# excamera/alfalfa

Hardware: AMD Instinct MI355X
Metric: 1080p macroblocks/s decode (bit-exact vs reference) (higher is better)
Workload: dtype u8

## Files before the change

### alfalfa_amd/__init__.py

```python
import os as _os

_os.environ.setdefault("GPU_MAX_HW_QUEUES", "16")

from .decoder import AlfalfaError, Context, Decoder, FilePlayer, Parser, Quality, psnr, read_ivf
```

### alfalfa_amd/capi.py

```python
import ctypes as C
import os

import numpy as np

from . import build as _build

AA_OK = 0
ERR_NAMES = {-1: "Invalid", -2: "Unsupported", -3: "LogicError", -4: "OutOfRange", -5: "HipError",
             -6: "NoDevice", -7: "BadArgument", -8: "NoMemory"}

AA_MB_HAS_NONZERO, AA_MB_HAS_Y2, AA_MB_INTER, AA_MB_SKIP, AA_MB_LF_SKIP_INNER = 1, 2, 4, 8, 16

MB_INFO_DTYPE = np.dtype([("y_mode", "u1"), ("uv_mode", "u1"), ("ref_frame", "u1"), ("segment_id", "u1"),
                          ("flags", "u1"), ("lf_level", "u1"), ("split_partition", "u1"), ("reserved", "u1"),
                          ("nz_mask", "<u4"), ("coeff_index", "<u4"), ("u", "u1", (64,))])
assert MB_INFO_DTYPE.itemsize == 80


class FrameHeader(C.Structure):
    _fields_ = [(n, C.c_uint8) for n in (
        "key_frame", "show_frame", "loop_filter_level", "sharpness_level", "num_dct_partitions",
        "segmentation_enabled", "filter_adjustments_enabled", "refresh_last", "refresh_golden",
        "refresh_alternate", "copy_buffer_to_golden", "copy_buffer_to_alternate", "sign_bias_golden",
        "sign_bias_alternate", "q_index", "has_intra_mb")] + [
        ("mb_width", C.c_uint16), ("mb_height", C.c_uint16), ("width", C.c_uint16), ("height", C.c_uint16),
        ("quant", (C.c_uint16 * 6) * 4), ("num_macroblocks", C.c_uint32), ("num_coeff_blocks", C.c_uint32),
        ("num_intra_mbs", C.c_uint32), ("compressed_size", C.c_uint32)]

    def as_dict(self):
        d = {n: getattr(self, n) for n, _ in self._fields_ if n != "quant"}
        d["quant"] = [[self.quant[s][k] for k in range(6)] for s in range(4)]
        return d


class FrameIn(C.Structure):
    _fields_ = [("stream", C.c_void_p), ("data", C.c_char_p), ("size", C.c_size_t)]


class KernelStats(C.Structure):
    _fields_ = [("recon_inter_ms", C.c_double), ("recon_intra_ms", C.c_double), ("loopfilter_ms", C.c_double),
                ("recon_inter_launches", C.c_uint64), ("recon_intra_launches", C.c_uint64),
                ("loopfilter_launches", C.c_uint64), ("macroblocks", C.c_uint64),
                ("parse_headers_ms", C.c_double), ("parse_tokens_ms", C.c_double), ("parse_launches", C.c_uint64),
                ("parsed_macroblocks", C.c_uint64), ("recon_split_ms", C.c_double), ("recon_split_launches", C.c_uint64),
                ("pool_waits", C.c_uint64), ("pool_wait_ms", C.c_double), ("parse_wait_ms", C.c_double),
                ("bind_wait_ms", C.c_double), ("alloc_ms", C.c_double), ("slab_mallocs", C.c_uint64),
                ("token_steps", C.c_uint64), ("token_frames", C.c_uint64), ("worker_launches", C.c_uint64), ("worker_wgs", C.c_uint64),
                ("worker_retires", C.c_uint64), ("heap_grows", C.c_uint64), ("heap_mapped_bytes", C.c_uint64), ("nomem_retries", C.c_uint64), ("frames_evicted", C.c_uint64), ("host_routed_frames", C.c_uint64),
                ("row_handoff_stale_polls", C.c_uint64), ("row_handoff_rereads", C.c_uint64), ("packed_frames", C.c_uint64), ("packed_words", C.c_uint64), ("packed_blocks", C.c_uint64),
                ("host_batch_ms", C.c_double), ("host_batch_parse_wall_ms", C.c_double), ("host_batch_parse_cpu_ms", C.c_double), ("host_batch_arena_ms", C.c_double),
                ("pinned_allocs", C.c_uint64)]


class CtxInfo(C.Structure):
    _fields_ = [(n, C.c_uint64) for n in ("memory_limit_bytes", "pool_bytes", "pool_free_bytes", "pool_pending_bytes", "heap_mapped_bytes", "heap_limit_bytes", "heap_used_bytes",
                                          "pinned_host_bytes")] + [
        (n, C.c_uint32) for n in ("heap_is_virtual", "token_lanes_per_workgroup", "token_workgroups_capacity", "token_workgroups_alive",
                                  "token_lane_lds_bytes", "token_workgroup_lds_bytes", "jobs_waiting", "compute_units")] + [
        ("heap_free_chunks", C.c_int32), ("lanes_starved", C.c_uint32), ("token_profile", C.c_uint64 * 8),
        ("packed_coefficients", C.c_uint32), ("lane_per_partition", C.c_uint32), ("clock_mhz", C.c_uint32), ("host_share_ms", C.c_uint32), ("host_rate_kb_per_ms", C.c_uint32), ("reserved1", C.c_uint32), ("stream_concurrency", C.c_uint32), ("streams_needed", C.c_uint32),
        ("host_waited_parse_ms", C.c_uint32), ("host_waited_compute_ms", C.c_uint32)]


AA_RGB_U8_HWC3, AA_RGB_U8_HWC4, AA_RGB_U8_CHW, AA_RGB_F16_CHW, AA_RGB_BF16_CHW, AA_RGB_F32_CHW = range(6)


class RgbTarget(C.Structure):
    _fields_ = [("dst", C.c_void_p), ("row_stride", C.c_int64), ("plane_stride", C.c_int64)]


AA_QUALITY_Y, AA_QUALITY_YUV = 1, 3


class QualityRef(C.Structure):
    _fields_ = [("y", C.c_void_p), ("u", C.c_void_p), ("v", C.c_void_p), ("y_stride", C.c_int64), ("uv_stride", C.c_int64)]


class AlfalfaError(RuntimeError):

    def __init__(self, code, message):
        super().__init__("%s: %s" % (ERR_NAMES.get(code, str(code)), message))
        self.code, self.kind, self.message = code, ERR_NAMES.get(code, str(code)), message


_P = C.c_void_p
_U8P = C.POINTER(C.c_uint8)
SYMBOLS = [
    ("aa_last_error", C.c_char_p, []), ("aa_abi_version", C.c_int, []), ("aa_runtime_prepare", C.c_int, []), ("aa_host_cpus", C.c_int, []), ("aa_device_count", C.c_int, []),
    ("aa_parser_create", C.c_int, [C.c_uint16, C.c_uint16, C.POINTER(_P)]), ("aa_parser_destroy", None, [_P]),
    ("aa_parser_parse", C.c_int, [_P, C.c_char_p, C.c_size_t, C.POINTER(FrameHeader), _P, _P]),
    ("aa_parser_get_probs", C.c_int, [_P, _U8P]), ("aa_parser_set_error_concealment", C.c_int, [_P, C.c_int]),
    ("aa_parse_frame_tag", C.c_int, [C.c_char_p, C.c_size_t, C.c_uint16, C.c_uint16, C.c_int] + [C.POINTER(C.c_int)] * 4),
    ("aa_stream_set_error_concealment", C.c_int, [_P, C.c_int]), ("aa_stream_error_concealment", C.c_int, [_P]),
    ("aa_parser_get_segmentation", C.c_int, [_P, C.POINTER(C.c_int), C.POINTER(C.c_int), C.POINTER(C.c_int8), C.POINTER(C.c_int8), _U8P]),
    ("aa_parser_get_filter_adjustments", C.c_int, [_P, C.POINTER(C.c_int), C.POINTER(C.c_int8), C.POINTER(C.c_int8)]),
    ("aa_parser_serialize_state", C.c_int, [_P, _P, C.c_size_t, _P]), ("aa_parser_deserialize_state", C.c_int, [_P, _P, C.c_size_t]),
    ("aa_stream_serialize", C.c_int, [_P, _P, C.c_size_t, _P]), ("aa_stream_deserialize", C.c_int, [_P, _P, C.c_size_t]),
    ("aa_parser_state_size", C.c_size_t, [_P]), ("aa_parser_export_state", C.c_int, [_P, _P, C.c_size_t]),
    ("aa_parser_import_state", C.c_int, [_P, C.c_char_p, C.c_size_t]),
    ("aa_stream_state_size", C.c_size_t, [_P]), ("aa_stream_export_state", C.c_int, [_P, _P, C.c_size_t]),
    ("aa_stream_import_state", C.c_int, [_P, C.c_char_p, C.c_size_t]),
    ("aa_stream_export_raster", C.c_int, [_P, C.c_int, _P, _P, _P]),
    ("aa_ctx_create", C.c_int, [C.c_int, C.POINTER(_P)]), ("aa_ctx_destroy", None, [_P]), ("aa_ctx_sync", C.c_int, [_P]),
    ("aa_ctx_memory", C.c_int, [_P, C.POINTER(C.c_size_t), C.POINTER(C.c_size_t)]),
    ("aa_ctx_set_memory_limit", C.c_int, [_P, C.c_size_t]), ("aa_ctx_set_packed_coefficients", C.c_int, [_P, C.c_int]), ("aa_ctx_set_host_share_ms", C.c_int, [_P, C.c_double]), ("aa_ctx_set_lane_per_partition", C.c_int, [_P, C.c_int]), ("aa_ctx_get_info", C.c_int, [_P, C.POINTER(CtxInfo)]),
    ("aa_ctx_set_schedule", C.c_int, [_P, C.c_int]), ("aa_ctx_clear_error", C.c_int, [_P]), ("aa_ctx_compute_stream", _P, [_P]), ("aa_ctx_copy_stream", _P, [_P]),
    ("aa_stream_create", C.c_int, [_P, C.c_uint16, C.c_uint16, C.POINTER(_P)]), ("aa_stream_destroy", None, [_P]),
    ("aa_stream_parse", C.c_int, [_P, C.c_char_p, C.c_size_t, C.POINTER(C.c_int), C.POINTER(FrameHeader)]),
    ("aa_stream_append_records", C.c_int, [_P, C.POINTER(FrameHeader), _P, _P, C.POINTER(C.c_int)]),
    ("aa_stream_upload", C.c_int, [_P]), ("aa_stream_release_staging", C.c_int, [_P]),
    ("aa_decode_batch", C.c_int, [_P, C.POINTER(_P), C.c_int, C.POINTER(C.c_int)]),
    ("aa_stream_decode", C.c_int, [_P, C.c_char_p, C.c_size_t, C.POINTER(C.c_int), C.POINTER(C.c_int)]),
    ("aa_submit_frames", C.c_int, [_P, C.POINTER(FrameIn), C.c_int, C.POINTER(C.c_int), C.c_int]),
    ("aa_submit_frames_ex", C.c_int, [_P, C.POINTER(FrameIn), C.c_int, C.POINTER(C.c_int), C.c_int, C.c_uint]),
    ("aa_launch_tokens", C.c_int, [_P, C.c_int, C.POINTER(C.c_int)]),
    ("aa_ssim_host", C.c_int, [C.c_char_p, C.c_char_p, C.c_int, C.c_int, C.POINTER(C.c_double)]),
    ("aa_stream_lf_search", C.c_int, [_P, C.c_char_p, C.c_size_t, C.c_void_p, C.c_int, C.c_int, C.POINTER(C.c_int), C.POINTER(C.c_double),
                                      C.POINTER(C.c_double), C.c_void_p]),
    ("aa_stream_frame_header", C.c_int, [_P, C.c_int, C.POINTER(FrameHeader)]),
    ("aa_stream_read_records", C.c_int, [_P, C.c_int, _P, _P, C.c_size_t]),
    ("aa_stream_frame_count", C.c_int, [_P]), ("aa_stream_release_before", C.c_int, [_P, C.c_int]),
    ("aa_stream_rewind", C.c_int, [_P]), ("aa_stream_rewind_to", C.c_int, [_P, C.c_int]),
    ("aa_stream_download", C.c_int, [_P, C.c_int, _P, _P, _P]),
    ("aa_pinned_alloc", C.c_int, [_P, C.c_size_t, C.POINTER(_P)]), ("aa_pinned_free", None, [_P]),
    ("aa_stream_download_async", C.c_int, [_P, C.c_int, _P, _P, _P]), ("aa_stream_download_wait", C.c_int, [_P]),
    ("aa_download_batch_async", C.c_int, [_P, C.POINTER(_P), C.c_int, C.POINTER(C.c_int), _P, C.c_size_t]), ("aa_ctx_download_wait", C.c_int, [_P]), ("aa_ctx_download_wait_until", C.c_int, [_P, C.c_int]),
    ("aa_stream_raster_device", C.c_int, [_P, C.c_int, C.POINTER(_P), C.POINTER(_P), C.POINTER(_P)]),
    ("aa_render_rgb_async", C.c_int, [_P, C.POINTER(_P), C.c_int, C.POINTER(C.c_int), C.c_int, C.POINTER(RgbTarget),
                                      C.POINTER(C.c_double), C.POINTER(C.c_double), _P]),
    ("aa_quality_batch_async", C.c_int, [_P, C.POINTER(_P), C.c_int, C.POINTER(C.c_int), C.POINTER(QualityRef), C.c_int, _P, _P, _P]),
    ("aa_stream_references", C.c_int, [_P, C.POINTER(C.c_int), C.POINTER(C.c_int), C.POINTER(C.c_int)]),
    ("aa_stream_reference_slots", C.c_int, [_P, C.POINTER(C.c_int)]),
    ("aa_stream_import_reference", C.c_int, [_P, _P, _P, _P]),
    ("aa_stream_import_reference_host", C.c_int, [_P, _P, _P, _P]),
    ("aa_parser_state_hash", C.c_int, [_P, C.POINTER(C.c_uint64)]), ("aa_stream_state_hash", C.c_int, [_P, C.POINTER(C.c_uint64)]),
    ("aa_stream_raster_hash", C.c_int, [_P, C.c_int, C.POINTER(C.c_uint64)]),
    ("aa_stream_decoder_hash", C.c_int, [_P, C.POINTER(C.c_uint64), C.POINTER(C.c_uint64)]),
    ("aa_stream_minihash", C.c_int, [_P, C.POINTER(C.c_uint32)]),
    ("aa_stream_release_frame", C.c_int, [_P, C.c_int]),
    ("aa_stream_set_references", C.c_int, [_P, C.POINTER(_P * 3), C.POINTER(C.c_int)]),
    ("aa_stream_reference_device", C.c_int, [_P, C.c_int, C.POINTER(_P), C.POINTER(_P), C.POINTER(_P)]),
    ("aa_stream_reference_download", C.c_int, [_P, C.c_int, _P, _P, _P]),
    ("aa_raster_geometry", None, [C.c_uint16, C.c_uint16, C.POINTER(C.c_uint32), C.POINTER(C.c_uint32)]),
    ("aa_ctx_profile", C.c_int, [_P, C.c_int]), ("aa_ctx_kernel_stats", C.c_int, [_P, C.POINTER(KernelStats), C.c_int]),
]

_lib = None


def lib():
    global _lib
    if _lib is None:
        path = _build.LIB
        if os.environ.get("ALFALFA_AMD_LIB"):
            path = os.environ["ALFALFA_AMD_LIB"]
        elif _build.stale():
            if os.path.exists(_build.HIPCC):
                _build.build()
            elif not os.path.exists(path):
                raise RuntimeError("libalfalfa_amd.so is missing and hipcc is not available: there is no CPU fallback")
        for name in ("libhsa-runtime64.so", "libamdhip64.so"):
            try:
                C.CDLL(name, mode=C.RTLD_GLOBAL)
            except OSError:
                pass
        L = C.CDLL(path)
        for name, restype, argtypes in SYMBOLS:
            fn = getattr(L, name)
            fn.restype, fn.argtypes = restype, argtypes
        L.aa_runtime_prepare()
        _lib = L
    return _lib


def check(rc):
    if rc != AA_OK:
        raise AlfalfaError(rc, lib().aa_last_error().decode("utf-8", "replace"))


def device_count():
    return lib().aa_device_count()


def raster_geometry(width, height):
    pw, ph = C.c_uint32(), C.c_uint32()
    lib().aa_raster_geometry(width, height, C.byref(pw), C.byref(ph))
    return pw.value, ph.value
```

### alfalfa_amd/csrc/device_types.h

```cpp
#pragma once
#include <stdint.h>

#include "../../include/alfalfa_amd.h"

struct aa_dev_frame {
  uint8_t * cur[3];
  const uint8_t * ref[4][3];
  const aa_mb_info * mbs;
  const int16_t * coeffs;
  const unsigned long long * intra_rows;
  uint16_t quant[4][6];
  uint16_t mbw, mbh;
  uint8_t key_frame;
  uint8_t loop_filter_level;
  uint8_t sharpness;
  uint8_t has_intra;
  uint32_t packed;
};

struct aa_raster_binding {
  aa_dev_frame * job;
  uint8_t * cur[3];
  const uint8_t * ref[3][3];
};

struct aa_gather_job {
  const uint8_t * src;
  size_t bytes;
};

struct aa_rgb_job {
  const uint8_t * plane[3];
  uint8_t * dst;
  int64_t row_stride, plane_stride;
  uint32_t stride_y, stride_c;
  uint32_t width, height;
  uint32_t groups;
  uint32_t pad;
};

#define AA_QUALITY_STRIP_ROWS 8
#define AA_QUALITY_CHUNK_WINDOWS 480
struct aa_quality_job {
  const uint8_t * a, * b;
  int64_t stride_a, stride_b;
  uint32_t w4, h4;
  uint32_t groups;
  uint32_t strips, chunks;
  uint32_t pad;
  uint64_t out_off;
};

#define AA_MAX_XCD 16

#define AA_SYNC_WS_DUMP 140
#define AA_SYNC_WS_RESCUES 132
struct aa_sync_ws {
  int error;
  int where[3];
  int dump[AA_SYNC_WS_DUMP];
  int ticket[AA_MAX_XCD];
  int progress[1];
};
#define AA_SYNC_WS_ZERO_FROM ( 16 + 4 * AA_SYNC_WS_DUMP )

#define AA_MAX_BATCH 480

struct aa_frame_list {
  const aa_dev_frame * f[AA_MAX_BATCH];
};

struct aa_seg_stream { uint8_t * map; uint32_t first, count; };

#define AA_MAX_WORKER_GRIDS 16
struct aa_tok_mirror {
  uint32_t seq;
  uint32_t q_head, q_publish, q_reserve;
  int32_t pool_avail;
  uint32_t pool_starving;
  uint32_t exited[AA_MAX_WORKER_GRIDS];
  unsigned long long prof[8];
};

namespace aa {
struct ParseJob;
struct TokQueue; struct CoeffPool; struct Heap;
int launch_parse_mb_headers( const ParseJob * jobs, const uint32_t * order, int n, void * stream );
int launch_segment_fixup( const ParseJob * jobs, const aa_seg_stream * streams, int n_streams, const uint32_t * order, void * stream );
void token_worker_shape( uint32_t lane_bytes, int n_cus, int * lanes_out, uint32_t * lds_out, int * wgs_per_cu_out );
int launch_token_workers( TokQueue * q, unsigned long long * slots, const Heap & heap, uint32_t * exited, const uint32_t * retire, uint32_t gen, uint32_t spread,
                          unsigned long long * prof, unsigned long long linger_ticks, int wgs, int lanes, uint32_t lane_bytes, uint32_t lds, bool packed, uint32_t mp_hint, void * stream,
                          uint32_t * cu_slots = nullptr, uint32_t cu_cap = 0 );
#define AA_CU_SLOTS ( 16 * 256 )
int launch_enqueue_jobs( TokQueue * q, unsigned long long * slots, const ParseJob * jobs, const uint32_t * order, int n, void * stream );
int launch_pool_push_range( const Heap & heap, uint32_t first, uint32_t count, void * stream );
int launch_pool_free_lists( const Heap & heap, const uint32_t * const * lists, int n, void * stream );
int launch_mirror_counters( const TokQueue * q, const CoeffPool * pool, const uint32_t * exited, int n_grids, const unsigned long long * prof, aa_tok_mirror * out, uint32_t seq, void * stream );
int launch_recon_inter4( const aa_frame_list & list, int n, unsigned max_mbs, void * stream );
int launch_recon_inter( const aa_frame_list & list, int n, unsigned max_mbs, bool split_only, void * stream );
int launch_recon_intra_diagonal( const aa_frame_list & list, int n, int diagonal, int row_lo, int rows, void * stream );
int launch_loopfilter_diagonal( const aa_frame_list & list, int n, int diagonal, int row_lo, int rows, void * stream );
int launch_recon_intra4( const aa_frame_list & list, int n_groups, int mbh_max, aa_sync_ws * ws, int n_xcd, void * stream );
int launch_loopfilter_rows4( const aa_frame_list & list, int n_groups, int mbh_max, int mbw_max, aa_sync_ws * ws, uint8_t * boundary, int n_xcd, void * stream );
int launch_probe_xcds( int * out16, int blocks, void * stream );
int launch_probe_concurrency( uint32_t * counter, uint32_t * seen, uint32_t n, unsigned long long timeout_ticks, int slot, void * stream );
int launch_bind_rasters( const aa_raster_binding * b, int n, void * stream );
int launch_gather_rasters( const aa_gather_job * jobs, int n, uint8_t * staging, size_t stride, size_t max_bytes, void * stream );
int launch_render_rgb( const aa_rgb_job * jobs, int n, int format, const uint32_t * table, uint32_t max_threads, void * stream );
int launch_lf_relevel( const aa_mb_info * src, aa_mb_info * dst, unsigned nmb, uint32_t levels, void * stream );
int launch_ssim_windows( const uint8_t * a, const uint8_t * b, int width, int height, float * out, void * stream );
int launch_quality( const aa_quality_job * jobs, int n_planes, uint32_t max_blocks, float * group_values, double * ssim, unsigned long long * sse, void * stream );
}
```

### alfalfa_amd/csrc/kernels.hip

```cpp
#include <hip/hip_runtime.h>
#include <algorithm>
#include <cstddef>

#include <cstdlib>

#include "device_types.h"
#include "vp8_math.hh"
#include "coeff_pack.hh"
#include "recon_inl.hh"

namespace aa {
namespace {
using namespace recon;

constexpr int kLanes = 64;

enum : int { DC_PRED, V_PRED, H_PRED, TM_PRED, B_PRED, NEARESTMV, NEARMV, ZEROMV, NEWMV, SPLITMV };

struct alignas( 16 ) ResidualLds {
  union {
    int16_t cf[25][16];
    int16_t res[24][16];
  };
  int16_t im[24][16];
  uint8_t map[32];
};

__device__ void compute_residual( const aa_mb_info & mb, const aa_dev_frame & f, ResidualLds & L, const int lane )
{
  uint32_t * z = reinterpret_cast<uint32_t *>( &L.cf[0][0] );
  for ( int i = lane; i < 200; i += kLanes ) z[i] = 0;
  const uint32_t mask = mb.nz_mask;
  if ( lane < 25 && ( ( mask >> lane ) & 1u ) ) L.map[lane == 24 ? 0 : __popc( mask & ( ( 1u << lane ) - 1u ) ) + static_cast<int>( mask >> 24 )] = static_cast<uint8_t>( lane );
  __syncthreads();
  const uint16_t * q = f.quant[mb.segment_id & 3];
  if ( f.packed ) {
    const int16_t * const w = f.coeffs + ( static_cast<size_t>( mb.reserved ) << 32 | mb.coeff_index );
    uint16_t * const scr = reinterpret_cast<uint16_t *>( &L.im[0][0] );
    if ( lane < 25 ) scr[lane] = ( ( mask >> lane ) & 1u ) ? static_cast<uint16_t>( w[lane] ) : 0u;
    __syncthreads();
    if ( lane < 25 ) {
      uint32_t off = pack::kMaskSlots;
      if ( lane != 24 ) { off += __popc( scr[24] ); for ( int b = 0; b < lane; b++ ) off += __popc( scr[b] ); }
      scr[32 + lane] = static_cast<uint16_t>( off );
    }
    __syncthreads();
    for ( int k = lane; k < 25 * 16; k += kLanes ) {
      const int blk = k >> 4, e = k & 15;
      const uint32_t m = scr[blk], zz = pack::zigzag_of( e );
      if ( ( m >> zz ) & 1u ) {
        const int base = blk < 16 ? 0 : ( blk < 24 ? 4 : 2 );
        L.cf[blk][e] = static_cast<int16_t>( dequant( w[scr[32 + blk] + __popc( m & ( ( 1u << zz ) - 1u ) )], q[base + ( e ? 1 : 0 )] ) );
      }
    }
  } else {
    const int n = __popc( mask ) * 16;
    const int16_t * src = f.coeffs + static_cast<size_t>( mb.coeff_index ) * 16;
    for ( int k = lane; k < n; k += kLanes ) {
      const int blk = L.map[k >> 4], e = k & 15;
      const int base = blk < 16 ? 0 : ( blk < 24 ? 4 : 2 );
      L.cf[blk][e] = static_cast<int16_t>( dequant( src[k], q[base + ( e ? 1 : 0 )] ) );
    }
  }
  __syncthreads();
  if ( mb.flags & AA_MB_HAS_Y2 ) {
    if ( lane < 4 ) {
      const Quad v = iwht_pass1( L.cf[24][lane], L.cf[24][lane + 4], L.cf[24][lane + 8], L.cf[24][lane + 12] );
      L.im[0][lane] = static_cast<int16_t>( v.v0 ); L.im[0][lane + 4] = static_cast<int16_t>( v.v1 );
      L.im[0][lane + 8] = static_cast<int16_t>( v.v2 ); L.im[0][lane + 12] = static_cast<int16_t>( v.v3 );
    }
    __syncthreads();
    if ( lane < 4 ) {
      const int o = lane * 4;
      const Quad v = iwht_pass2( L.im[0][o], L.im[0][o + 1], L.im[0][o + 2], L.im[0][o + 3] );
      L.cf[o + 0][0] = static_cast<int16_t>( v.v0 ); L.cf[o + 1][0] = static_cast<int16_t>( v.v1 );
      L.cf[o + 2][0] = static_cast<int16_t>( v.v2 ); L.cf[o + 3][0] = static_cast<int16_t>( v.v3 );
    }
    __syncthreads();
  }
  for ( int t = lane; t < 96; t += kLanes ) {
    const int blk = t >> 2, i = t & 3;
    const Quad v = idct_pass1( L.cf[blk][i], L.cf[blk][i + 4], L.cf[blk][i + 8], L.cf[blk][i + 12] );
    L.im[blk][i * 4 + 0] = static_cast<int16_t>( v.v0 ); L.im[blk][i * 4 + 1] = static_cast<int16_t>( v.v1 );
    L.im[blk][i * 4 + 2] = static_cast<int16_t>( v.v2 ); L.im[blk][i * 4 + 3] = static_cast<int16_t>( v.v3 );
  }
  __syncthreads();
  for ( int t = lane; t < 96; t += kLanes ) {
// ... 720 lines not shown
#pragma unroll
      for ( int k = 0; k < 4; k++ ) { a[k] = *reinterpret_cast<const uint32_t *>( &S.y[0][16 + 4 * k] ); sa += absdiff_sum4( a[k] ); }
#pragma unroll
      for ( int i = 0; i < 16; i++ ) sl += S.y[i + 1][15];
      const int dc = bigpred_dc( sa, sl, row > 0, col > 0, 4 );
      const int corner = S.y[0][15], left = S.y[r + 1][15];
      uint32_t o[4];
#pragma unroll
      for ( int k = 0; k < 4; k++ ) o[k] = bigpred_x4( y_mode, a[k], left, corner, dc, has_res, &S.res[( r >> 2 ) * 4 + k][( r & 3 ) * 4] );
      *reinterpret_cast<uint4 *>( Y + static_cast<size_t>( y0 + r ) * pw + x0 ) = make_uint4( o[0], o[1], o[2], o[3] );
    }
    if ( __any( bp ) ) {
#pragma unroll
      for ( int b = 0; b < 16; b++ ) {
        const int bx = b & 3, by = b >> 2;
        const int ar = by * 4, ac = bx * 4 + 15;
        if ( bp ) {
          const uint32_t word = by == 0 ? bm.x : ( by == 1 ? bm.y : ( by == 2 ? bm.z : bm.w ) );
          const int mode = ( word >> ( 8 * bx ) ) & 0xFF;
          const uint32_t e = L.tab[mode * 16 + l];
          const uint8_t * const org = &S.y[ar][ac];
          const int lift = bx == 3 ? ar * 48 : 0;
          const int e0 = org[static_cast<int>( e & 0xFF ) - ( ( e >> 24 ) & 1 ? lift : 0 )];
          const int e1 = org[static_cast<int>( ( e >> 8 ) & 0xFF ) - ( ( e >> 25 ) & 1 ? lift : 0 )];
          const int e2 = org[static_cast<int>( ( e >> 16 ) & 0xFF ) - ( ( e >> 26 ) & 1 ? lift : 0 )];
          const uint32_t above4 = *reinterpret_cast<const uint32_t *>( &S.y[ar][ac + 1] );
          const int dc = ( absdiff_sum4( above4 ) + S.y[ar + 1][ac] + S.y[ar + 2][ac] + S.y[ar + 3][ac] + S.y[ar + 4][ac] + 4 ) >> 3;
          int v = bpred_eval( e >> 27, e0, e1, e2, dc );
          if ( has_res ) v = clamp255( v + S.res[b][l] );
          S.y[ar + 1 + ( l >> 2 )][ac + 1 + ( l & 3 )] = static_cast<uint8_t>( v );
        }
        __syncthreads();
      }
      if ( bp ) *reinterpret_cast<uint4 *>( Y + static_cast<size_t>( y0 + l ) * pw + x0 ) = *reinterpret_cast<const uint4 *>( &S.y[l + 1][16] );
    }
    __syncthreads();
  }
  publish_progress( frame_on && l == 0 && !row_done, &progress[row], mbw );
}

__global__ __launch_bounds__( kLanes ) void k_recon_intra4( const aa_frame_list list, const int n_groups, const int mbh_max, aa_sync_ws * ws, const int n_xcd )
{
  __builtin_amdgcn_s_setprio( 3 );

  __shared__ Intra4Lds L;
  __shared__ int s_ticket;
  for ( int i = threadIdx.x; i < 160; i += kLanes ) {
    const uint32_t e = bpred_entry( i >> 4, i & 3, ( i >> 2 ) & 3 );
    uint32_t packed = ( e >> 24 ) << 27;
    for ( int k = 0; k < 3; k++ ) {
      const uint32_t idx = ( e >> ( 8 * k ) ) & 0xFF;
      packed |= ( idx < 4 ? ( 4 - idx ) * 48 : idx - 4 ) << ( 8 * k );
      packed |= ( idx >= 9 ? 1u : 0u ) << ( 24 + k );
    }
    L.tab[i] = packed;
  }
  const int xcc = xcc_id();
  if ( xcc >= n_xcd ) { if ( threadIdx.x == 0 ) atomicExch( &ws->error, 3 ); return; }
  for ( ;; ) {
    const int t = take_ticket( ws, xcc, &s_ticket, threadIdx.x );
    const int mine = xcc < n_groups ? ( n_groups - xcc + n_xcd - 1 ) / n_xcd : 0;
    if ( t >= mine * mbh_max ) return;
    recon_intra4_row( list, ( t % mine ) * n_xcd + xcc, t / mine, mbh_max, ws, L, xcc );
  }
}

struct alignas( 16 ) Inter4Slot {
  alignas( 16 ) int16_t res[24][16];
  union {
    struct {
      alignas( 16 ) uint8_t wy[21][24];
      uint8_t wc[2][13][16];
    };
    alignas( 16 ) uint8_t pred[384];
  };
  union {
    alignas( 16 ) uint8_t ty[16][24];
    alignas( 16 ) int16_t y2[32];
  };
  alignas( 16 ) uint8_t tc[2][8][16];
};
struct alignas( 16 ) Inter4Lds { Inter4Slot slot[4]; uint32_t taps[16]; };
static_assert( offsetof( Inter4Slot, wc ) == offsetof( Inter4Slot, wy ) + 21 * 24, "wy and wc must be contiguous" );

__device__ __forceinline__ void recon_inter4_body( const aa_dev_frame & f, const unsigned bq, const unsigned max_quads, Inter4Lds & L )
{
  const int lane = threadIdx.x, slot = lane >> 4, l = lane & 15;
  Inter4Slot & S = L.slot[slot];
  if ( lane < 16 ) {
    uint32_t a, b; pack_taps( lane >> 1, a, b ); L.taps[lane] = ( lane & 1 ) ? b : a;
  }
  const unsigned total = static_cast<unsigned>( f.mbw ) * f.mbh;
  const unsigned chunk = ( max_quads + 7u ) >> 3;
  const unsigned qi = ( bq & 7u ) * chunk + ( bq >> 3 );
  const unsigned mi = qi * 4u + slot;
  const int mbw = f.mbw, pw = mbw * 16, ph = f.mbh * 16, cw = pw >> 1, ch = ph >> 1;
  bool on = qi < max_quads && mi < total;
  const aa_mb_info * const mb = f.mbs + ( on ? mi : 0u );
  uint4 hd = make_uint4( 0, 0, 0, 0 ); uint32_t mvw = 0;
  if ( on ) { hd = *reinterpret_cast<const uint4 *>( mb ); mvw = *reinterpret_cast<const uint32_t *>( &mb->u.mv[0][0] ); }
  const int y_mode = hd.x & 0xFF, ref_frame = ( hd.x >> 16 ) & 3, segment = ( hd.x >> 24 ) & 3, flags = hd.y & 0xFF;
  const uint32_t nz_mask = hd.z, coeff_index = hd.w;
  on = on && ( flags & AA_MB_INTER ) && y_mode != SPLITMV;
  if ( !__any( on ) ) return;
  const int col = on ? static_cast<int>( mi % static_cast<unsigned>( mbw ) ) : 0, row = on ? static_cast<int>( mi / static_cast<unsigned>( mbw ) ) : 0;
  const bool has_res = on && ( flags & AA_MB_HAS_NONZERO );
  const bool has_y2 = has_res && ( flags & AA_MB_HAS_Y2 );
  const uint8_t * const * ref = f.ref[on ? ref_frame : 1];
  const uint8_t * const ref_y = ref[0], * const ref_u = ref[1], * const ref_v = ref[2];
  const int mvx = static_cast<int16_t>( mvw & 0xFFFFu ), mvy = static_cast<int>( mvw ) >> 16;
  const int cmx = chroma_mv( 4 * mvx ), cmy = chroma_mv( 4 * mvy );
  const int sxy = col * 16 + ( mvx >> 3 ) - 2, syy = row * 16 + ( mvy >> 3 ) - 2;
  const int sxc = col * 8 + ( cmx >> 3 ) - 2, syc = row * 8 + ( cmy >> 3 ) - 2;
  const int axy = sxy & ~3, axc = sxc & ~3;
  const bool inside = sxy >= 0 && syy >= 0 && axy + 24 <= pw && syy + 21 <= ph && sxc >= 0 && syc >= 0 && axc + 16 <= cw && syc + 13 <= ch;
  const bool fast = on && inside;
  uint32_t wreg[15];
  const int l6 = l / 6, lm = l - 6 * l6;
  const uint8_t * const wy0 = ref_y + static_cast<ptrdiff_t>( syy ) * pw + axy;
  const uint8_t * const wu0 = ref_u + static_cast<ptrdiff_t>( syc ) * cw + axc;
  const uint8_t * const wv0 = ref_v + static_cast<ptrdiff_t>( syc ) * cw + axc;
#pragma unroll
  for ( int k = 0; k < 15; k++ ) {
    const int i = l + 16 * k;
    wreg[k] = 0;
    if ( fast ) {
      if ( k < 7 || ( k == 7 && i < 126 ) ) {
        const int carry = lm + ( 4 * k ) % 6 >= 6 ? 1 : 0;
        const int r = l6 + 2 * k + ( 4 * k ) / 6 + carry, d = lm + ( 4 * k ) % 6 - 6 * carry;
        wreg[k] = *reinterpret_cast<const uint32_t *>( wy0 + static_cast<ptrdiff_t>( r ) * pw + d * 4 );
      } else if ( i < 230 ) {
        const int j = i - 126, pl = j >= 52 ? 1 : 0, e = j - 52 * pl;
        wreg[k] = *reinterpret_cast<const uint32_t *>( ( pl ? wv0 : wu0 ) + static_cast<ptrdiff_t>( e >> 2 ) * cw + ( e & 3 ) * 4 );
      }
    }
  }

  residual_x4( S, f, has_res, has_y2, nz_mask, coeff_index, hd.y >> 24, segment, l );

  {
    uint32_t * flat = reinterpret_cast<uint32_t *>( &S.wy[0][0] );
    if ( fast ) {
#pragma unroll
      for ( int k = 0; k < 15; k++ ) { const int i = l + 16 * k; if ( i < 230 ) flat[i] = wreg[k]; }
    }
    if ( __any( on && !inside ) ) {
      if ( on && !inside ) {
        uint8_t * by = &S.wy[0][0];
        for ( int i = l; i < 21 * 24; i += 16 ) {
          const int r = i / 24, c = i % 24;
          by[i] = ref_y[static_cast<size_t>( clampi( syy + r, 0, ph - 1 ) ) * pw + clampi( sxy + c, 0, pw - 1 )];
        }
        uint8_t * bc = &S.wc[0][0][0];
        for ( int i = l; i < 2 * 13 * 16; i += 16 ) {
          const int pl = i / 208, e = i % 208, r = e >> 4, c = e & 15;
          bc[i] = ( pl ? ref_v : ref_u )[static_cast<size_t>( clampi( syc + r, 0, ch - 1 ) ) * cw + clampi( sxc + c, 0, cw - 1 )];
        }
      }
    }
  }
  const int oy = inside ? ( sxy & 3 ) : 0, oc = inside ? ( sxc & 3 ) : 0;
  __syncthreads();

  const bool luma_general = __any( on && ( ( mvx | mvy ) & 7 ) != 0 ), chroma_general = __any( on && ( ( cmx | cmy ) & 7 ) != 0 );
  const uint8_t * const wyb = &S.wy[0][0]; const uint8_t * const wcb = &S.wc[0][0][0];
  uint8_t * const tyb = &S.ty[0][0]; uint8_t * const tcb = &S.tc[0][0][0];
  if ( on && luma_general ) {
    const int frac = mvx & 7;
    const uint32_t t0 = L.taps[2 * frac], t1 = L.taps[2 * frac + 1];
#pragma unroll
    for ( int k = 0; k < 6; k++ ) {
      const int t = l + 16 * k;
      if ( k == 5 && t >= 84 ) continue;
      const int r = t >> 2, g = t & 3;
      const uint8_t * sp = wyb + r * 24 + g * 4;
      const uint32_t o4 = sixtap_x4_lane( *reinterpret_cast<const uint32_t *>( sp ), *reinterpret_cast<const uint32_t *>( sp + 4 ), *reinterpret_cast<const uint32_t *>( sp + 8 ), oy, frac, t0, t1 );
      uint8_t * tb = tyb + ( g * 4 ) * 24 + r;
      tb[0] = static_cast<uint8_t>( o4 ); tb[24] = static_cast<uint8_t>( o4 >> 8 ); tb[48] = static_cast<uint8_t>( o4 >> 16 ); tb[72] = static_cast<uint8_t>( o4 >> 24 );
    }
  }
  if ( on && chroma_general ) {
    const int frac = cmx & 7;
    const uint32_t t0 = L.taps[2 * frac], t1 = L.taps[2 * frac + 1];
#pragma unroll
    for ( int k = 0; k < 4; k++ ) {
      const int j = l + 16 * k;
      if ( k == 3 && j >= 52 ) continue;
      const int pl = j >= 26 ? 1 : 0, e = j - 26 * pl, r = e >> 1, g = e & 1;
      const uint8_t * sp = wcb + pl * 208 + r * 16 + g * 4;
      const uint32_t o4 = sixtap_x4_lane( *reinterpret_cast<const uint32_t *>( sp ), *reinterpret_cast<const uint32_t *>( sp + 4 ), *reinterpret_cast<const uint32_t *>( sp + 8 ), oc, frac, t0, t1 );
      uint8_t * tb = tcb + pl * 128 + ( g * 4 ) * 16 + r;
      tb[0] = static_cast<uint8_t>( o4 ); tb[16] = static_cast<uint8_t>( o4 >> 8 ); tb[32] = static_cast<uint8_t>( o4 >> 16 ); tb[48] = static_cast<uint8_t>( o4 >> 24 );
    }
  }
  uint4 copy_y = make_uint4( 0, 0, 0, 0 ); uint2 copy_c = make_uint2( 0, 0 );
  if ( !luma_general && on ) {
    const uint2 * rp = reinterpret_cast<const uint2 *>( wyb + ( l + 2 ) * 24 );
    const uint2 a = rp[0], b = rp[1], c = rp[2];
    const bool q = oy + 2 >= 4; const int sft = ( oy + 2 ) & 3;
    const uint32_t e0 = q ? a.y : a.x, e1 = q ? b.x : a.y, e2 = q ? b.y : b.x, e3 = q ? c.x : b.y, e4 = q ? c.y : c.x;
    copy_y = make_uint4( __builtin_amdgcn_alignbyte( e1, e0, sft ), __builtin_amdgcn_alignbyte( e2, e1, sft ),
                         __builtin_amdgcn_alignbyte( e3, e2, sft ), __builtin_amdgcn_alignbyte( e4, e3, sft ) );
  }
  if ( !chroma_general && on ) {
    const int pl = l >> 3, r = l & 7;
    const uint2 * rp = reinterpret_cast<const uint2 *>( wcb + pl * 208 + ( r + 2 ) * 16 );
    const uint2 a = rp[0], b = rp[1];
    const bool q = oc + 2 >= 4; const int sft = ( oc + 2 ) & 3;
    const uint32_t e0 = q ? a.y : a.x, e1 = q ? b.x : a.y, e2 = q ? b.y : b.x;
    copy_c = make_uint2( __builtin_amdgcn_alignbyte( e1, e0, sft ), __builtin_amdgcn_alignbyte( e2, e1, sft ) );
  }
  __syncthreads();
  if ( !luma_general && on ) *reinterpret_cast<uint4 *>( S.pred + l * 16 ) = copy_y;
  if ( !chroma_general && on ) *reinterpret_cast<uint2 *>( S.pred + 256 + ( l >> 3 ) * 64 + ( l & 7 ) * 8 ) = copy_c;
  if ( on && luma_general ) {
    const int frac = mvy & 7;
    const uint32_t t0 = L.taps[2 * frac], t1 = L.taps[2 * frac + 1];
#pragma unroll
    for ( int k = 0; k < 4; k++ ) {
      const int t = l + 16 * k, c = t >> 2, i = t & 3;
      const uint8_t * sp = tyb + c * 24 + i * 4;
      const uint32_t o4 = sixtap_x4_lane( *reinterpret_cast<const uint32_t *>( sp ), *reinterpret_cast<const uint32_t *>( sp + 4 ), *reinterpret_cast<const uint32_t *>( sp + 8 ), 0, frac, t0, t1 );
      uint8_t * pb = S.pred + ( i * 4 ) * 16 + c;
      pb[0] = static_cast<uint8_t>( o4 ); pb[16] = static_cast<uint8_t>( o4 >> 8 ); pb[32] = static_cast<uint8_t>( o4 >> 16 ); pb[48] = static_cast<uint8_t>( o4 >> 24 );
    }
  }
  if ( on && chroma_general ) {
    const int frac = cmy & 7;
    const uint32_t t0 = L.taps[2 * frac], t1 = L.taps[2 * frac + 1];
#pragma unroll
    for ( int k = 0; k < 2; k++ ) {
      const int j = l + 16 * k, pl = j >> 4, c = ( j >> 1 ) & 7, i = j & 1;
      const uint8_t * sp = tcb + pl * 128 + c * 16 + i * 4;
      const uint32_t o4 = sixtap_x4_lane( *reinterpret_cast<const uint32_t *>( sp ), *reinterpret_cast<const uint32_t *>( sp + 4 ), *reinterpret_cast<const uint32_t *>( sp + 8 ), 0, frac, t0, t1 );
      uint8_t * pb = S.pred + 256 + pl * 64 + ( i * 4 ) * 8 + c;
      pb[0] = static_cast<uint8_t>( o4 ); pb[8] = static_cast<uint8_t>( o4 >> 8 ); pb[16] = static_cast<uint8_t>( o4 >> 16 ); pb[24] = static_cast<uint8_t>( o4 >> 24 );
    }
  }
  __syncthreads();

  if ( on ) {
    uint32_t o[4];
#pragma unroll
    for ( int k = 0; k < 4; k++ ) {
      const uint32_t p4 = *reinterpret_cast<const uint32_t *>( S.pred + l * 16 + 4 * k );
      const uint32_t out = has_res ? add_residual_x4( p4, &S.res[( l >> 2 ) * 4 + k][( l & 3 ) * 4] ) : p4;
      o[k] = out;
    }
    *reinterpret_cast<uint4 *>( f.cur[0] + static_cast<size_t>( row * 16 + l ) * pw + col * 16 ) = make_uint4( o[0], o[1], o[2], o[3] );
    const int pl = l >> 3, r = l & 7;
    uint32_t oc2[2];
#pragma unroll
    for ( int k = 0; k < 2; k++ ) {
      const uint32_t p4 = *reinterpret_cast<const uint32_t *>( S.pred + 256 + pl * 64 + r * 8 + 4 * k );
      const uint32_t out = has_res ? add_residual_x4( p4, &S.res[16 + pl * 4 + ( r >> 2 ) * 2 + k][( r & 3 ) * 4] ) : p4;
      oc2[k] = out;
    }
    *reinterpret_cast<uint2 *>( f.cur[1 + pl] + static_cast<size_t>( row * 8 + r ) * cw + col * 8 ) = make_uint2( oc2[0], oc2[1] );
  }
}

__global__ __launch_bounds__( kLanes ) void k_recon_inter4( const aa_frame_list list, const unsigned max_quads )
{
  __builtin_amdgcn_s_setprio( 3 );

  __shared__ Inter4Lds L;
  recon_inter4_body( *list.f[blockIdx.y], blockIdx.x, max_quads, L );
}

constexpr int kStripMbs = 8;
constexpr int kStripRow = 16 + 16 * kStripMbs;
constexpr int kStripRpi = 16 / kStripMbs;
static_assert( ( kStripRow / 16 ) % 2 == 1, "odd multiple of 16: consecutive rows start on different banks" );
struct alignas( 16 ) LfStrip {
  uint8_t c[12][kStripRow];
  uint8_t y[20][kStripRow];
  uint8_t halo_y[16][4];
  uint8_t halo_c[2][8][4];
  uint8_t pad[32];
};
struct alignas( 16 ) LfStripLds { LfStrip slot[4]; };

__device__ __forceinline__ uint64_t load_u64_shared( const uint8_t * p )
{
  return __hip_atomic_load( reinterpret_cast<const uint64_t *>( p ), __ATOMIC_RELAXED, __HIP_MEMORY_SCOPE_AGENT );
}

__device__ __forceinline__ void lf_edges_pk( pk2 ( &v )[20], const LfParamsPk & P, const pk2 g0, const pk2 g1, const pk2 g23 )
{
  if ( __any( g0 != 0u ) ) lf_edge_pk( P, true, g0, v[0], v[1], v[2], v[3], v[4], v[5], v[6], v[7] );
  if ( __any( g1 != 0u ) ) {
    lf_edge_pk( P, false, g1, v[4], v[5], v[6], v[7], v[8], v[9], v[10], v[11] );
    if ( __any( g23 != 0u ) ) {
      lf_edge_pk( P, false, g23, v[8], v[9], v[10], v[11], v[12], v[13], v[14], v[15] );
      lf_edge_pk( P, false, g23, v[12], v[13], v[14], v[15], v[16], v[17], v[18], v[19] );
    }
  }
}

__device__ __forceinline__ void loopfilter_strip_row( const aa_frame_list & list, const int group, const int row, const int mbh_max, const int mbw_max,
                                                       aa_sync_ws * ws, uint8_t * bnd, LfStripLds & S, const int dbg, const int home_xcc )
{
  const int lane = threadIdx.x, slot = lane >> 4, l = lane & 15;
  const aa_dev_frame & f0 = *list.f[group * 4];
  const int mbh = f0.mbh;
  if ( row >= mbh ) return;
  const aa_dev_frame * const fp = list.f[group * 4 + slot];
  const bool frame_on = fp != nullptr && fp->loop_filter_level != 0;
  if ( !__any( frame_on ) ) return;
  const aa_dev_frame & f = fp ? *fp : f0;
  LfStrip & T = S.slot[slot];
  int * const progress = ws->progress + group * mbh_max;
  const int mbw = f0.mbw, pw = mbw * 16, cw = pw >> 1;
  const int y0 = row * 16, cy0 = row * 8;
  const int sharp = f.sharpness; const bool key = f.key_frame;
  const bool last_row = row == mbh - 1;
  const bool luma = l < 8;
  const int k8 = l & 7, cp = k8 >> 2, cj = k8 & 3;
  uint8_t * const vrow = luma ? &T.y[4 + 2 * l][16] : &T.c[4 + 2 * cj][16 + 8 * kStripMbs * cp];
  uint8_t * const vhalo = luma ? &T.halo_y[2 * l][0] : &T.halo_c[cp][2 * cj][0];
  uint8_t * const hcol = luma ? &T.y[0][16 + 2 * l] : &T.c[0][16 + 8 * kStripMbs * cp + 2 * cj];
  const int mbstep = luma ? 16 : 8;
  const int brow = l / kStripMbs, bchunk = l % kStripMbs;
  uint8_t * const gy = f.cur[0] + static_cast<size_t>( y0 + brow ) * pw + 16 * bchunk;
  uint8_t * const gu = f.cur[1] + static_cast<size_t>( cy0 + brow ) * cw + 8 * bchunk;
  uint8_t * const gv = f.cur[2] + static_cast<size_t>( cy0 + brow ) * cw + 8 * bchunk;
  uint8_t * const sy = &T.y[4 + brow][16 + 16 * bchunk];
  uint8_t * const sc = &T.c[4 + brow][16 + 8 * bchunk];
  const int bl = l & 7, bq = ( bl - 4 ) & 3;
  uint8_t * const bsrc = bl < 4 ? &T.y[16 + bl][16] : &T.c[8 + 2 * ( bq & 1 )][16 + 8 * kStripMbs * ( bq >> 1 )];
  uint8_t * const btop = bl < 4 ? &T.y[bl][16] : &T.c[2 * ( bq & 1 )][16 + 8 * kStripMbs * ( bq >> 1 )];
  const int bstep = bl < 4 ? 16 : 8;
  const size_t bnd_row = ( static_cast<size_t>( group * 4 + slot ) * mbh_max + row ) * mbw_max;
  uint8_t * const bnd_own = bnd + bnd_row * 128 + 16 * bl;
  const uint8_t * const bnd_top = bnd + ( bnd_row - mbw_max ) * 128 + 16 * bl;
  const int fq = l >> 2, fr = l & 3;
  const int fix_off = fq == 0 ? 16 * fr + 12 : 64 + 32 * ( fq - 1 ) + 8 * fr + 4;
  uint8_t * const fix_src0 = fq == 0 ? &T.halo_y[12 + fr][0] : &T.halo_c[( fq - 1 ) & 1][4 + fr][0];
  uint8_t * const fix_srck = fq == 0 ? &T.y[16 + fr][16 - 4] : &T.c[8 + fr][16 + 8 * kStripMbs * ( ( fq - 1 ) & 1 ) - 4];
  const int fix_step = fq == 0 ? 16 : 8;
  uint8_t * const fy = f.cur[0] + static_cast<size_t>( y0 + l ) * pw - 4;
  uint8_t * const fc = f.cur[1 + ( l >> 3 )] + static_cast<size_t>( cy0 + ( l & 7 ) ) * cw - 4;
  const aa_mb_info * const mbrow = f.mbs + static_cast<size_t>( row ) * mbw;

  const int n_strips = ( mbw + kStripMbs - 1 ) / kStripMbs;
  uint4 py[kStripMbs]; uint2 pc[kStripMbs];
#pragma unroll
  for ( int i = 0; i < kStripMbs; i++ ) { py[i] = make_uint4( 0, 0, 0, 0 ); pc[i] = make_uint2( 0, 0 ); }
  auto prefetch = [&]( const int s ) {
    const bool in = frame_on && !( dbg & 2 ) && s * kStripMbs + bchunk < mbw;
// ... 324 lines not shown
      const uint32_t p = ( wa[k >> 2] >> ( 8 * ( k & 3 ) ) ) & 255u, q = ( wb[k >> 2] >> ( 8 * ( k & 3 ) ) ) & 255u;
      s1 += p; s2 += q; ss += p * p + q * q; s12 += p * q;
    }
  }
  const int i1 = static_cast<int>( s1 ), i2 = static_cast<int>( s2 ), iss = static_cast<int>( ss ), i12 = static_cast<int>( s12 );
  const int c1 = 416, c2 = 235963;
  const int vars = iss * 64 - i1 * i1 - i2 * i2, covar = i12 * 64 - i1 * i2;
  const float num = __fmul_rn( static_cast<float>( 2 * i1 * i2 + c1 ), static_cast<float>( 2 * covar + c2 ) );
  const float den = __fmul_rn( static_cast<float>( i1 * i1 + i2 * i2 + c1 ), static_cast<float>( vars + c2 ) );
  out[static_cast<size_t>( y ) * ( w4 - 1 ) + x] = __fdiv_rn( num, den );
}

__global__ __launch_bounds__( 256 ) void k_lf_relevel( const aa_mb_info * src, aa_mb_info * dst, unsigned nmb, uint32_t levels )
{
  const unsigned i = blockIdx.x * blockDim.x + threadIdx.x;
  if ( i >= nmb ) return;
  const uint4 * s = reinterpret_cast<const uint4 *>( src + i );
  uint4 * d = reinterpret_cast<uint4 *>( dst + i );
  uint4 head = s[0];
  const uint32_t seg = ( head.x >> 24 ) & 3u;
  head.y = ( head.y & 0xFFFF00FFu ) | ( ( ( levels >> ( 8 * seg ) ) & 255u ) << 8 );
  d[0] = head;
  for ( int k = 1; k < 5; k++ ) d[k] = s[k];
}
static_assert( sizeof( aa_mb_info ) == 80, "k_lf_relevel copies five 16-byte pieces" );

int launch_lf_relevel( const aa_mb_info * src, aa_mb_info * dst, unsigned nmb, uint32_t levels, void * stream )
{
  hipLaunchKernelGGL( k_lf_relevel, dim3( ( nmb + 255 ) / 256 ), dim3( 256 ), 0, static_cast<hipStream_t>( stream ), src, dst, nmb, levels );
  return static_cast<int>( hipGetLastError() );
}

int launch_ssim_windows( const uint8_t * a, const uint8_t * b, int width, int height, float * out, void * stream )
{
  const int w4 = width >> 2, h4 = height >> 2;
  if ( w4 < 2 || h4 < 2 ) return static_cast<int>( hipErrorInvalidValue );
  hipLaunchKernelGGL( k_ssim_windows, dim3( ( w4 - 1 + 255 ) / 256, h4 - 1 ), dim3( 256 ), 0, static_cast<hipStream_t>( stream ), a, b, width, w4, h4, out );
  return static_cast<int>( hipGetLastError() );
}

int launch_gather_rasters( const aa_gather_job * jobs, int n, uint8_t * staging, size_t stride, size_t max_bytes, void * stream )
{
  const unsigned per = static_cast<unsigned>( std::min<size_t>( 64, std::max<size_t>( 1, max_bytes / ( 256 * 16 * 4 ) ) ) );
  for ( int base = 0; base < n; base += 32768 ) {
    const int cnt = std::min( 32768, n - base );
    hipLaunchKernelGGL( k_gather_rasters, dim3( per, cnt ), dim3( 256 ), 0, static_cast<hipStream_t>( stream ), jobs + base, staging + stride * base, stride );
    if ( hipError_t e = hipGetLastError() ) return static_cast<int>( e );
  }
  return 0;
}

int launch_render_rgb( const aa_rgb_job * jobs, int n, int format, const uint32_t * table, uint32_t max_threads, void * stream )
{
  const unsigned blocks = ( max_threads + 255u ) / 256u;
  const hipStream_t st = static_cast<hipStream_t>( stream );
  for ( int base = 0; base < n; base += 32768 ) {
    const dim3 grid( blocks, std::min( 32768, n - base ) );
    switch ( format ) {
      case AA_RGB_U8_HWC3: hipLaunchKernelGGL( k_render_rgb<AA_RGB_U8_HWC3>, grid, dim3( 256 ), 0, st, jobs + base, table ); break;
      case AA_RGB_U8_HWC4: hipLaunchKernelGGL( k_render_rgb<AA_RGB_U8_HWC4>, grid, dim3( 256 ), 0, st, jobs + base, table ); break;
      case AA_RGB_U8_CHW: hipLaunchKernelGGL( k_render_rgb<AA_RGB_U8_CHW>, grid, dim3( 256 ), 0, st, jobs + base, table ); break;
      case AA_RGB_F16_CHW: hipLaunchKernelGGL( k_render_rgb<AA_RGB_F16_CHW>, grid, dim3( 256 ), 0, st, jobs + base, table ); break;
      case AA_RGB_BF16_CHW: hipLaunchKernelGGL( k_render_rgb<AA_RGB_BF16_CHW>, grid, dim3( 256 ), 0, st, jobs + base, table ); break;
      case AA_RGB_F32_CHW: hipLaunchKernelGGL( k_render_rgb<AA_RGB_F32_CHW>, grid, dim3( 256 ), 0, st, jobs + base, table ); break;
      default: return static_cast<int>( hipErrorInvalidValue );
    }
    if ( hipError_t e = hipGetLastError() ) return static_cast<int>( e );
  }
  return 0;
}

int launch_bind_rasters( const aa_raster_binding * b, int n, void * stream )
{
  hipLaunchKernelGGL( k_bind_rasters, dim3( ( n + 63 ) / 64 ), dim3( 64 ), 0, static_cast<hipStream_t>( stream ), b, n );
  return static_cast<int>( hipGetLastError() );
}

int launch_recon_inter( const aa_frame_list & list, int n, unsigned max_mbs, bool split_only, void * stream )
{
  const unsigned blocks = ( ( max_mbs + 7u ) >> 3 ) * 8u;
  hipLaunchKernelGGL( k_recon_inter, dim3( blocks, n ), dim3( kLanes ), 0, static_cast<hipStream_t>( stream ), list, max_mbs, split_only ? 1 : 0 );
  return static_cast<int>( hipGetLastError() );
}
int launch_recon_inter4( const aa_frame_list & list, int n, unsigned max_mbs, void * stream )
{
  const unsigned quads = ( max_mbs + 3u ) >> 2;
  const unsigned blocks = ( ( quads + 7u ) >> 3 ) * 8u;
  hipLaunchKernelGGL( k_recon_inter4, dim3( blocks, n ), dim3( kLanes ), 0, static_cast<hipStream_t>( stream ), list, quads );
  return static_cast<int>( hipGetLastError() );
}
int launch_recon_intra_diagonal( const aa_frame_list & list, int n, int diagonal, int row_lo, int rows, void * stream )
{
  hipLaunchKernelGGL( k_recon_intra, dim3( rows, n ), dim3( kLanes ), 0, static_cast<hipStream_t>( stream ), list, diagonal, row_lo );
  return static_cast<int>( hipGetLastError() );
}
int launch_loopfilter_diagonal( const aa_frame_list & list, int n, int diagonal, int row_lo, int rows, void * stream )
{
  hipLaunchKernelGGL( k_loopfilter, dim3( rows, n ), dim3( kLanes ), 0, static_cast<hipStream_t>( stream ), list, diagonal, row_lo );
  return static_cast<int>( hipGetLastError() );
}
static int lf_debug_bits()
{
  static const int bits = [] { const char * e = std::getenv( "ALFALFA_AMD_LF_DEBUG" ); return e ? std::atoi( e ) : 0; }();
  return bits;
}
static unsigned test_lds_pad()
{
  static const unsigned pad = [] { const char * e = std::getenv( "ALFALFA_AMD_TEST_LDS_PAD" ); return e ? static_cast<unsigned>( std::atoi( e ) ) : 0u; }();
  return pad;
}
int launch_loopfilter_rows4( const aa_frame_list & list, int n_groups, int mbh_max, int mbw_max, aa_sync_ws * ws, uint8_t * boundary, int n_xcd, void * stream )
{
  hipLaunchKernelGGL( k_loopfilter_rows4, dim3( n_xcd * ( ( n_groups + n_xcd - 1 ) / n_xcd ) * mbh_max ), dim3( kLanes ), test_lds_pad(), static_cast<hipStream_t>( stream ), list, n_groups, mbh_max, mbw_max, ws, boundary, n_xcd, lf_debug_bits() );
  hipLaunchKernelGGL( k_check_tickets, dim3( 1 ), dim3( 64 ), 0, static_cast<hipStream_t>( stream ), ws, n_groups, mbh_max, n_xcd );
  return static_cast<int>( hipGetLastError() );
}
int launch_recon_intra4( const aa_frame_list & list, int n_groups, int mbh_max, aa_sync_ws * ws, int n_xcd, void * stream )
{
  hipLaunchKernelGGL( k_recon_intra4, dim3( n_xcd * ( ( n_groups + n_xcd - 1 ) / n_xcd ) * mbh_max ), dim3( kLanes ), test_lds_pad(), static_cast<hipStream_t>( stream ), list, n_groups, mbh_max, ws, n_xcd );
  hipLaunchKernelGGL( k_check_tickets, dim3( 1 ), dim3( 64 ), 0, static_cast<hipStream_t>( stream ), ws, n_groups, mbh_max, n_xcd );
  return static_cast<int>( hipGetLastError() );
}
int launch_probe_concurrency( uint32_t * counter, uint32_t * seen, uint32_t n, unsigned long long timeout_ticks, int slot, void * stream )
{
  hipLaunchKernelGGL( k_probe_concurrency, dim3( 1 ), dim3( 64 ), 0, static_cast<hipStream_t>( stream ), counter, seen, n, timeout_ticks, slot );
  return static_cast<int>( hipGetLastError() );
}
int launch_probe_xcds( int * out16, int blocks, void * stream )
{
  hipLaunchKernelGGL( k_probe_xcds, dim3( blocks ), dim3( kLanes ), 0, static_cast<hipStream_t>( stream ), out16 );
  return static_cast<int>( hipGetLastError() );
}

}
```

### alfalfa_amd/csrc/parse_kernels.hip

```cpp
#include <hip/hip_runtime.h>

#include <algorithm>

#include "device_types.h"
#include "tok_fsm.hh"
#include "coeff_pack.hh"

#ifndef AA_WORKER_PRIO
#define AA_WORKER_PRIO 3
#endif

namespace {

using aa::ParseJob;

__global__ __launch_bounds__( 64 ) void k_parse_mb_headers( const ParseJob * jobs, const uint32_t * order, int n, int lanes )
{
  __builtin_amdgcn_s_setprio( 2 );

  __shared__ aa::HeaderTables s_tables;
  __shared__ aa::HeaderParams s_params[16];
  const int lane = threadIdx.x;
  for ( uint32_t k = lane; k < sizeof( aa::HeaderTables ) / 4; k += 64 ) reinterpret_cast<uint32_t *>( &s_tables )[k] = reinterpret_cast<const uint32_t *>( &aa::kHeaderTables )[k];
  const int slot = blockIdx.x * lanes + lane;
  const bool mine = lane < lanes && lane < 16 && slot < n;
  const ParseJob * Jp = mine ? &jobs[order[slot]] : nullptr;
  if ( Jp ) {
    const uint32_t * src = reinterpret_cast<const uint32_t *>( static_cast<const aa::HeaderParams *>( &Jp->fp ) );
    for ( uint32_t k = 0; k < sizeof( aa::HeaderParams ) / 4; k++ ) reinterpret_cast<uint32_t *>( &s_params[lane] )[k] = src[k];
  }
  __syncthreads();
  if ( !Jp ) return;
  const ParseJob & J = *Jp;
  if ( J.nmb == 0 ) return;
  const aa::HeaderParams & fp = s_params[lane];
  const aa::HeaderTables & T = s_tables;
  aa::BoolReader32 bd;
  aa::BoolState st; st.bitpos = fp.bd_bitpos; st.range = fp.bd_range; st.active = fp.bd_active;
  bd.resume( J.data + fp.first_off, fp.first_size, st );
  const unsigned mbw = fp.mbw, mbh = fp.mbh;
  const unsigned words_per_row = ( mbw + 63 ) / 64;
  uint32_t intra = 0, split = 0;
  unsigned mi = 0;
  const uint32_t mp_stride = J.mp_stride, mp_base = J.flags_padded, nparts = fp.nparts;
  for ( unsigned row = 0; row < mbh; row++ ) {
    unsigned long long word = 0;
    const uint32_t mp_row = mp_stride ? mp_base + ( row % nparts ) * mp_stride + ( row / nparts ) * mbw : 0u;
    for ( unsigned col = 0; col < mbw; col++, mi++ ) {
      const uint8_t flags = aa::parse_mb_header( bd, fp, T, J.mbs, mi, col, row, static_cast<uint8_t *>( nullptr ) );
      J.mbflags[mi] = flags;
      if ( mp_stride ) J.mbflags[mp_row + col] = flags;
      if ( !( flags & AA_MB_INTER ) ) { intra++; word |= 1ull << ( col & 63 ); }
      else if ( J.mbs[mi].y_mode == aa::SPLITMV ) split = 1;
      if ( ( col & 63 ) == 63 || col + 1 == mbw ) { J.intra_rows[row * words_per_row + ( col >> 6 )] = word; word = 0; }
    }
  }
  J.summary->num_intra_mbs = intra;
  J.summary->has_split = split;
}

__global__ __launch_bounds__( 256 ) void k_segment_fixup( const ParseJob * jobs, const aa_seg_stream * streams, const uint32_t * order )
{
  const aa_seg_stream s = streams[blockIdx.x];
  for ( uint32_t k = 0; k < s.count; k++ ) {
    const uint32_t o = order[s.first + k];
    const ParseJob & J = jobs[o & 0x7FFFFFFFu];
    if ( !J.fp.seg_enabled || J.nmb == 0 ) continue;
    if ( o >> 31 ) {
      for ( uint32_t mi = threadIdx.x; mi < J.nmb; mi += blockDim.x ) s.map[mi] = 3;
      __syncthreads();
    }
    for ( uint32_t mi = threadIdx.x; mi < J.nmb; mi += blockDim.x ) aa::segment_fixup( J.fp, J.mbs[mi], s.map[mi] );
    __syncthreads();
  }
}

struct WorkerArgs {
  aa::TokQueue * q;
  unsigned long long * slots;
  aa::Heap heap;
  uint32_t * exited;
  const uint32_t * retire;
  uint32_t gen;
  uint32_t spread;
  unsigned long long * prof;
  unsigned long long linger_ticks;
  int lanes;
  uint32_t lane_bytes;
  uint32_t mp_hint;
  uint32_t * cu_slots;
  uint32_t cu_cap;
  int16_t * sink;
};

__device__ inline uint32_t queue_take( aa::TokQueue * q, uint32_t want, uint32_t spread, uint32_t * base )
{
  uint32_t h = AA_AT_LOAD( &q->head );
  for ( uint32_t tries = 0; ; tries++ ) {
    const uint32_t avail = AA_AT_LOAD( &q->publish ) - h;
    if ( static_cast<int32_t>( avail ) <= 0 ) return 0;
    const uint32_t share = ( avail + spread - 1u ) / spread;
    const uint32_t n = want < share ? want : share;
    uint32_t expect = h;
    if ( __hip_atomic_compare_exchange_strong( &q->head, &expect, h + n, __ATOMIC_RELAXED, __ATOMIC_RELAXED, __HIP_MEMORY_SCOPE_AGENT ) ) { *base = h; return n; }
    h = expect;
    const uint32_t r = ( blockIdx.x * 2654435761u + tries * 40503u ) >> 27;
    for ( uint32_t k = 0; k <= ( r & ( tries < 4 ? 3u : tries < 8 ? 15u : 31u ) ); k++ ) __builtin_amdgcn_s_sleep( 16 );
    if ( tries > 2048 ) h = AA_AT_LOAD( &q->head );
  }
}

__device__ inline int nth_set_bit( unsigned long long mask, uint32_t n )
{
  for ( uint32_t k = 0; k < n; k++ ) mask &= mask - 1ull;
  return __ffsll( static_cast<long long>( mask ) ) - 1;
}

template <bool PK, bool MP>
__global__ __launch_bounds__( 64 ) void k_token_workers( const WorkerArgs a )
{
  extern __shared__ __attribute__( ( aligned( 16 ) ) ) uint8_t smem[];
  const int lane = threadIdx.x;
#if AA_WORKER_PRIO
  __builtin_amdgcn_s_setprio( AA_WORKER_PRIO );
#endif
  uint32_t cu_slot = 0;
  if ( a.cu_slots ) {
    const uint32_t hw = __builtin_amdgcn_s_getreg( 4 | ( 8 << 6 ) | ( 7 << 11 ) ), xcc = __builtin_amdgcn_s_getreg( 20 | ( 0 << 6 ) | ( 3 << 11 ) );
    cu_slot = ( ( xcc & 15u ) << 8 ) | ( hw & 255u );
    uint32_t before = 0;
    if ( lane == 0 ) before = AA_AT_ADD( &a.cu_slots[cu_slot], 1u );
    before = __shfl( before, 0 );
    if ( before >= a.cu_cap ) {
      if ( lane == 0 ) { AA_AT_ADD( &a.cu_slots[cu_slot], 0xFFFFFFFFu ); AA_AT_ADD( &a.cu_slots[AA_CU_SLOTS - 1], 1u ); AA_AT_ADD( a.exited, 1u ); }
      return;
    }
// ... 291 lines not shown
```

### alfalfa_amd/csrc/runtime_ctx.inc

```

extern "C" {

const char * aa_last_error( void ) { return g_last_error.c_str(); }
int aa_host_cpus( void ) { return effective_cpus(); }
int aa_runtime_prepare( void )
{
  const bool was_set = std::getenv( "GPU_MAX_HW_QUEUES" ) != nullptr;
  setenv( "GPU_MAX_HW_QUEUES", "16", 0 );
  return was_set ? 1 : 0;
}
int aa_abi_version( void ) { return AA_ABI_VERSION; }
int aa_device_count( void ) { int n = 0; if ( hipGetDeviceCount( &n ) != hipSuccess ) return 0; return n; }

void aa_raster_geometry( uint16_t width, uint16_t height, uint32_t * pw, uint32_t * ph )
{
  if ( pw ) *pw = 16u * ( ( width + 15u ) / 16u );
  if ( ph ) *ph = 16u * ( ( height + 15u ) / 16u );
}

aa_status aa_parser_create( uint16_t width, uint16_t height, aa_parser ** out )
{
  if ( !out || !width || !height ) return fail( AA_ERR_ARGUMENT, "aa_parser_create: bad argument" );
  *out = new ( std::nothrow ) aa_parser( width, height );
  return *out ? AA_OK : fail( AA_ERR_ARGUMENT, "out of memory" );
// ... 115 lines not shown
    ctx->prio_low = lo;
    HIP_TRY( hipStreamCreateWithPriority( &ctx->compute, hipStreamNonBlocking, hi ) );
  }
  HIP_TRY( hipStreamCreateWithFlags( &ctx->copy, hipStreamNonBlocking ) );
  HIP_TRY( hipEventCreateWithFlags( &ctx->upload_done, hipEventDisableTiming ) );
  {
    size_t free_b = 0, total_b = 0;
    if ( hipMemGetInfo( &free_b, &total_b ) == hipSuccess && free_b ) ctx->pool_soft_limit = free_b / 8 * 7;
    (void) hipGetLastError();
  }
  if ( const char * e = getenv( "ALFALFA_AMD_PARSE_STREAMS" ) ) ctx->n_parse_streams = std::max( 1, std::min( aa_ctx::kMaxParseStreams, atoi( e ) ) );
  ctx->parse_streams.assign( ctx->n_parse_streams, nullptr );
  ctx->parse_idle.assign( ctx->n_parse_streams, nullptr );
  for ( auto & ps : ctx->parse_streams ) HIP_TRY( hipStreamCreateWithPriority( &ps, hipStreamNonBlocking, ctx->prio_low ) );
  for ( auto & e : ctx->parse_idle ) HIP_TRY( hipEventCreateWithFlags( &e, hipEventDisableTiming ) );
  if ( const char * e = std::getenv( "ALFALFA_AMD_SCHEDULE" ) ) ctx->schedule = std::string( e ) == "diagonal" ? 1 : 0;
  if ( const char * e = std::getenv( "ALFALFA_AMD_PACKED" ) ) ctx->tok.packed = atoi( e ) != 0;
  if ( const char * e = std::getenv( "ALFALFA_AMD_LANE_PER_PARTITION" ) ) ctx->tok.lane_per_partition = atoi( e ) != 0;
  if ( const char * e = std::getenv( "ALFALFA_AMD_HOST_SHARE_MS" ) ) ctx->host_share_ms = std::max( 0.0, atof( e ) );
  {
    int * d = nullptr; int h[AA_MAX_XCD] = {};
    HIP_TRY( hipMalloc( reinterpret_cast<void **>( &d ), sizeof h ) );
    HIP_TRY( hipMemsetAsync( d, 0, sizeof h, ctx->compute ) );
    const int e2 = aa::launch_probe_xcds( d, 2048, ctx->compute );
    if ( e2 ) { (void) hipFree( d ); return hip_fail( static_cast<hipError_t>( e2 ), "k_probe_xcds" ); }
    HIP_TRY( hipStreamSynchronize( ctx->compute ) );
    HIP_TRY( hipMemcpy( h, d, sizeof h, hipMemcpyDeviceToHost ) );
    (void) hipFree( d );
    int n_xcd = 0;
    while ( n_xcd < AA_MAX_XCD && h[n_xcd] > 0 ) n_xcd++;
    for ( int x = n_xcd; x < AA_MAX_XCD; x++ ) if ( h[x] ) return fail( AA_ERR_HIP, "unexpected XCC id layout on this device (ids are not 0..n-1)" );
    if ( n_xcd == 0 ) return fail( AA_ERR_HIP, "XCD probe kernel did not run" );
    for ( int x = 0; x < n_xcd; x++ ) ctx->xcd_share[x] = h[x];
    ctx->n_xcd = n_xcd;
    for ( int x = 0; x < n_xcd; x++ ) if ( h[x] * n_xcd * 2 < 2048 ) ctx->schedule = 1;
  }
  *out = ctx.release();
  return AA_OK;
}
static void ctx_free( aa_ctx * ctx );
void aa_ctx_destroy( aa_ctx * ctx )
{
  if ( !ctx ) return;
  if ( --ctx->refs == 0 ) ctx_free( ctx );
}
static void ctx_free( aa_ctx * ctx )
{
  (void) hipSetDevice( ctx->device );
  (void) tok_quiesce( ctx );
  host_lanes_stop( ctx );
  (void) hipStreamSynchronize( ctx->compute ); (void) hipStreamSynchronize( ctx->copy );
  for ( auto ps : ctx->parse_streams ) if ( ps ) { (void) hipStreamSynchronize( ps ); (void) hipStreamDestroy( ps ); }
  for ( auto e : ctx->parse_idle ) if ( e ) (void) hipEventDestroy( e );
  for ( auto & ee : ctx->epoch_events ) { if ( ee.compute ) (void) hipEventDestroy( ee.compute ); if ( ee.copy ) (void) hipEventDestroy( ee.copy ); }
  if ( ctx->last_seg_batch ) (void) hipEventDestroy( ctx->last_seg_batch );
  drain_profile( ctx );
  for ( auto e : ctx->free_events ) (void) hipEventDestroy( e );
  (void) hipEventDestroy( ctx->upload_done );
  if ( ctx->last_raster_download ) (void) hipEventDestroy( ctx->last_raster_download );
  for ( auto & bb : ctx->bind_bufs ) { if ( bb.host ) (void) hipHostFree( bb.host ); if ( bb.done ) (void) hipEventDestroy( bb.done ); }
  for ( auto & gb : ctx->gather_bufs ) { if ( gb.host ) (void) hipHostFree( gb.host ); if ( gb.done ) (void) hipEventDestroy( gb.done ); if ( gb.copied ) (void) hipEventDestroy( gb.copied ); }
  for ( auto & rb : ctx->rgb_bufs ) {
    if ( rb.host ) (void) hipHostFree( rb.host );
    if ( rb.dev ) (void) hipFree( rb.dev );
    for ( hipEvent_t e : { rb.done, rb.before, rb.after } ) if ( e ) (void) hipEventDestroy( e );
  }
  for ( auto & qb : ctx->quality_bufs ) {
    if ( qb.host ) (void) hipHostFree( qb.host );
    for ( hipEvent_t e : { qb.done, qb.before, qb.after } ) if ( e ) (void) hipEventDestroy( e );
  }
  if ( ctx->ws ) (void) hipFree( ctx->ws );
  if ( ctx->boundary ) (void) hipFree( ctx->boundary );
  tok_free( ctx );
  for ( auto & pc : ctx->pinned_pool ) (void) hipHostFree( pc.first );
  for ( uint8_t * slab : ctx->dev_slabs ) (void) hipFree( slab );
  (void) hipStreamDestroy( ctx->compute ); (void) hipStreamDestroy( ctx->copy );
  delete ctx;
}
static aa_status check_watchdog( aa_ctx * ctx )
{
  if ( !ctx->ws ) return AA_OK;
  int err = 0;
  HIP_TRY( hipMemcpy( &err, &ctx->ws->error, sizeof err, hipMemcpyDeviceToHost ) );
  if ( err == 3 ) return fail( AA_ERR_HIP, "row-pipelined kernel: a workgroup ran on an XCD outside the probed set (output is not valid)" );
  if ( err == 5 ) {
    int hdr[4] = {};
    (void) hipMemcpy( hdr, ctx->ws, sizeof hdr, hipMemcpyDeviceToHost );
    return fail( AA_ERR_HIP, "row-pipelined kernel: XCD " + std::to_string( hdr[1] ) + " handed out " + std::to_string( hdr[2] ) + " of its " + std::to_string( hdr[3] )
                               + " macroblock rows: no workgroup of the launch ran there (output is not valid); use the diagonal schedule on this device" );
  }
  if ( err == 4 ) {
    int hdr[4] = {};
    (void) hipMemcpy( hdr, ctx->ws, sizeof hdr, hipMemcpyDeviceToHost );
    return fail( AA_ERR_HIP, "row-pipelined kernel: a wave of unit " + std::to_string( hdr[1] ) + " row " + std::to_string( hdr[2] ) + " moved from XCD "
                               + std::to_string( hdr[3] >> 16 ) + " to XCD " + std::to_string( hdr[3] & 0xFFFF ) + " (context save/restore under queue oversubscription?): "
                               "the in-launch hand-off is only coherent inside one XCD (output is not valid)" );
  }
  if ( err ) {
    int hdr[4 + AA_SYNC_WS_DUMP + AA_MAX_XCD] = {};
    (void) hipMemcpy( hdr, ctx->ws, sizeof hdr, hipMemcpyDeviceToHost );
    std::string tickets, rows;
    for ( int x = 0; x < ctx->n_xcd; x++ ) tickets += ( x ? "," : "" ) + std::to_string( hdr[4 + AA_SYNC_WS_DUMP + x] );
    const int * dump = hdr + 4;
    for ( int r = 0; r < std::min( 128, dump[130] ); r++ ) rows += ( r ? "," : "" ) + std::to_string( dump[r] );
    return fail( AA_ERR_HIP, std::string( "row-pipelined kernel " ) + ( err == 1 ? "k_recon_intra4" : "k_loopfilter_rows4" )
                               + ": a bounded wait for the macroblock row above expired (output is not valid); first at unit " + std::to_string( hdr[1] )
                               + " row " + std::to_string( hdr[2] ) + ", needed " + std::to_string( hdr[3] >> 16 ) + " saw " + std::to_string( hdr[3] & 0xFFFF )
                               + " after " + std::to_string( dump[128] ) + " polls in " + std::to_string( dump[129] ) + " ms; columns done per row of that unit when it gave up: " + rows
                               + "; tickets handed out per XCD (last launch): " + tickets );
  }
  return AA_OK;
}
aa_status aa_ctx_sync( aa_ctx * ctx )
{
  if ( !ctx ) return fail( AA_ERR_ARGUMENT, "null ctx" );
  if ( aa_status st = set_device( ctx ) ) return st;
  HIP_TRY( hipStreamSynchronize( ctx->copy ) );
  for ( auto ps : ctx->parse_streams ) HIP_TRY( hipStreamSynchronize( ps ) );
  if ( aa_status st = tok_quiesce( ctx ) ) return st;
  { std::lock_guard<std::mutex> g( ctx->pool_mu ); flush_chunk_frees( ctx ); }
  HIP_TRY( hipStreamSynchronize( ctx->compute ) );
  return check_watchdog( ctx );
}
aa_status aa_ctx_memory( aa_ctx * ctx, size_t * free_bytes, size_t * total_bytes )
{
  if ( !ctx ) return fail( AA_ERR_ARGUMENT, "null ctx" );
  if ( aa_status st = set_device( ctx ) ) return st;
  size_t f = 0, t = 0;
  HIP_TRY( hipMemGetInfo( &f, &t ) );
  if ( free_bytes ) *free_bytes = f;
  if ( total_bytes ) *total_bytes = t;
  return AA_OK;
}
aa_status aa_ctx_set_memory_limit( aa_ctx * ctx, size_t bytes )
{
  if ( !ctx || !bytes ) return fail( AA_ERR_ARGUMENT, "aa_ctx_set_memory_limit: bad argument" );
  std::lock_guard<std::mutex> g( ctx->pool_mu );
  ctx->pool_soft_limit = bytes;
  if ( !ctx->tok.ready ) ctx->tok.heap_limit = 0;
  return AA_OK;
}
aa_status aa_ctx_get_info( aa_ctx * ctx, aa_ctx_info * out )
{
  if ( !ctx || !out ) return fail( AA_ERR_ARGUMENT, "null argument" );
  if ( aa_status st = set_device( ctx ) ) return st;
  std::memset( out, 0, sizeof *out );
  auto & T = ctx->tok;
  {
    std::lock_guard<std::mutex> g( ctx->pool_mu );
    collect_pending( ctx, false );
    out->memory_limit_bytes = ctx->pool_soft_limit; out->pool_bytes = ctx->pool_bytes; out->pinned_host_bytes = ctx->pinned_bytes;
    for ( auto & kv : ctx->dev_free ) out->pool_free_bytes += kv.first * kv.second.size();
    for ( auto & pf : ctx->pending_free ) out->pool_pending_bytes += pf.bytes;
    if ( ctx->cur_slab ) out->pool_free_bytes += kSlabBytes - ctx->slab_used;
    out->pool_free_bytes += ctx->compute_free_bytes;
    for ( auto & h : ctx->compute_hold ) out->pool_pending_bytes += h.second;
  }
  out->heap_mapped_bytes = T.heap_mapped; out->heap_limit_bytes = T.heap_va;
  out->heap_used_bytes = static_cast<uint64_t>( std::max<int64_t>( 0, T.chunks_committed ) ) * kChunkBytesHeap;
  out->heap_is_virtual = T.vmm ? 1u : 0u;
  out->packed_coefficients = T.packed ? 1u : 0u;
  out->lane_per_partition = T.lane_per_partition ? 1u : 0u;
  out->token_lanes_per_workgroup = static_cast<uint32_t>( T.lanes ); out->token_workgroups_capacity = static_cast<uint32_t>( T.cap_wgs );
  out->token_lane_lds_bytes = T.lane_bytes; out->token_workgroup_lds_bytes = T.lds;
  out->compute_units = static_cast<uint32_t>( T.n_cus );
  out->host_share_ms = static_cast<uint32_t>( ctx->host_share_ms + 0.5 );
// ... 137 lines not shown
```

### alfalfa_amd/csrc/runtime_decode.inc

```
extern "C" {

static aa_status resolve_summary( aa_stream * s, FrameRec & r )
{
  if ( !r.summary_pending ) return AA_OK;
  aa_ctx * ctx = s->ctx;
  auto & T = ctx->tok;
  Batch * b = r.batch;
  if ( !b || !r.summary ) return fail( AA_ERR_LOGIC, "frame records were released before the frame was decoded" );
  if ( b->tokens_pending ) if ( aa_status st = launch_tokens_of( ctx, b ) ) return st;
  volatile aa::FrameSummary * sum = r.summary;
  for ( int attempt = 0; ; attempt++ ) {
    if ( aa_status st = tok_wait_done( ctx, sum ) ) return st;
    if ( sum->status != aa::TOK_NO_MEMORY ) break;
    ctx->stats.nomem_retries++;
    const uint32_t worst = aa::chunk_list_entries( r.hdr.num_macroblocks, T.lane_per_partition ? 8u : 1u );
    {
      std::lock_guard<std::mutex> g( ctx->pool_mu );
      if ( !r.chunks_returned ) { T.pending_lists.push_back( r.chunk_list ); r.chunks_returned = true; T.chunks_committed -= r.est_chunks; r.est_chunks = 0; }
      flush_chunk_frees( ctx );
      if ( !T.pending_lists.empty() ) return fail( AA_ERR_HIP, "k_pool_free_lists could not be launched" );
    }
    HIP_TRY( hipStreamSynchronize( ctx->compute ) );
    if ( aa_status st = tok_grow_heap( ctx, T.heap_mapped + static_cast<size_t>( worst ) * kChunkBytesHeap ) ) return st;
    if ( aa_status st = tok_refresh_mirror( ctx ) ) return st;
    if ( T.mirror_host->pool_avail < static_cast<int32_t>( worst ) ) {
      if ( aa_status st = tok_quiesce( ctx ) ) return st;
      if ( aa_status st = tok_refresh_mirror( ctx ) ) return st;
    }
    if ( T.mirror_host->pool_avail < static_cast<int32_t>( worst ) ) {
      int32_t have = T.mirror_host->pool_avail;
      std::lock_guard<std::mutex> g( ctx->pool_mu );
      for ( auto bi = T.batches.rbegin(); bi != T.batches.rend() && have < static_cast<int32_t>( worst ); ++bi ) {
        Batch * vb = *bi;
        volatile aa::FrameSummary * sums = reinterpret_cast<volatile aa::FrameSummary *>( vb->host + vb->summaries_off );
        for ( int i = vb->n - 1; i >= 0 && have < static_cast<int32_t>( worst ); i-- ) {
          if ( !vb->items[i].live ) continue;
          aa_stream * vs = vb->items[i].s;
          FrameRec & v = vs->frames[vb->items[i].frame];
          if ( &v == &r || vb->items[i].on_host || !v.enqueued || v.records_released || v.chunks_returned || !sums[i].done || vb->items[i].frame < vs->next_submit ) continue;
          T.pending_lists.push_back( v.chunk_list );
          have += static_cast<int32_t>( sums[i].num_chunks );
          v.chunks_returned = true; v.summary_pending = true;
          T.chunks_committed -= v.est_chunks; v.est_chunks = 0;
          sums[i].status = aa::TOK_NO_MEMORY;
          ctx->stats.frames_evicted++;
        }
      }
      flush_chunk_frees( ctx );
      if ( !T.pending_lists.empty() ) return fail( AA_ERR_HIP, "k_pool_free_lists could not be launched" );
    }
    HIP_TRY( hipStreamSynchronize( ctx->compute ) );
    if ( aa_status st = tok_refresh_mirror( ctx ) ) return st;
    if ( attempt >= 8 || T.mirror_host->pool_avail < static_cast<int32_t>( worst ) )
      return fail( AA_ERR_NO_MEMORY, "device parser: the coefficient heap is exhausted (" + std::to_string( T.heap_mapped >> 20 ) + " MiB mapped, "
                                     + std::to_string( T.mirror_host->pool_avail ) + " chunks free, this frame may need " + std::to_string( worst )
                                     + "): release decoded frames (aa_stream_release_before) or raise the limit (aa_ctx_set_memory_limit); the call can be repeated" );
    sum->status = 0; sum->done = 0; sum->num_chunks = 0;
    r.chunks_returned = false;
    r.est_chunks = worst; T.chunks_committed += worst;
    __atomic_thread_fence( __ATOMIC_SEQ_CST );
    if ( int e = aa::launch_enqueue_jobs( T.q, T.slots, r.parse_job, T.one_dev, 1, T.util ) ) return hip_fail( static_cast<hipError_t>( e ), "k_enqueue_jobs" );
    T.jobs_enqueued += 1;
    if ( std::find( T.inflight.begin(), T.inflight.end(), b ) == T.inflight.end() ) T.inflight.push_back( b );
    if ( aa_status st = tok_service( ctx ) ) return st;
  }
  if ( sum->status == aa::TOK_HOST_FAILED ) return fail( AA_ERR_HIP, "host lane: the frame's records could not be placed in device memory" );
  if ( sum->status == aa::TOK_STEP_BOUND ) return fail( AA_ERR_HIP, "device parser: a token lane exceeded the step bound of its frame size (records are not valid)" );
  r.hdr.num_coeff_blocks = sum->num_coeff_blocks;
  r.hdr.num_intra_mbs = sum->num_intra_mbs;
  r.hdr.has_intra_mb = sum->num_intra_mbs != 0;
  r.has_split = sum->has_split != 0;
  r.intra_diagonals.assign( r.hdr.mb_width + 2 * ( r.hdr.mb_height - 1 ), r.hdr.has_intra_mb ? 1 : 0 );
  T.chunks_committed += static_cast<int64_t>( sum->num_chunks ) - static_cast<int64_t>( r.est_chunks );
  r.est_chunks = sum->num_chunks;
  if ( r.hdr.compressed_size ) T.blocks_per_byte += 0.05 * ( static_cast<double>( sum->num_coeff_blocks ) / r.hdr.compressed_size - T.blocks_per_byte );
  if ( r.hdr.compressed_size && r.packed_pos ) T.words_per_byte += 0.05 * ( static_cast<double>( sum->packed_words ) / r.hdr.compressed_size - T.words_per_byte );
  if ( r.packed_pos ) { ctx->stats.packed_frames++; ctx->stats.packed_words += sum->packed_words; ctx->stats.packed_blocks += sum->num_coeff_blocks; }
  ctx->stats.token_steps += sum->steps; ctx->stats.token_frames++;
  r.summary_pending = false;
  return AA_OK;
}

aa_status aa_stream_frame_header( aa_stream * s, int fi, aa_frame_header * out )
{
  if ( !s || !out || fi < 0 || fi >= static_cast<int>( s->frames.size() ) ) return fail( AA_ERR_ARGUMENT, "aa_stream_frame_header: bad argument" );
  if ( aa_status st = set_device( s->ctx ) ) return st;
  if ( aa_status st = resolve_summary( s, s->frames[fi] ) ) return st;
  *out = s->frames[fi].hdr;
  return AA_OK;
}

aa_status aa_stream_read_records( aa_stream * s, int fi, aa_mb_info * mb_out, int16_t * coeff_out, size_t coeff_capacity_blocks )
{
  if ( !s || fi < 0 || fi >= static_cast<int>( s->frames.size() ) ) return fail( AA_ERR_ARGUMENT, "aa_stream_read_records: bad argument" );
  if ( aa_status st = set_device( s->ctx ) ) return st;
  FrameRec & r = s->frames[fi];
  if ( r.records_released ) return fail( AA_ERR_LOGIC, "aa_stream_read_records: frame records were released" );
  if ( aa_status st = resolve_summary( s, r ) ) return st;
  if ( aa_status st = aa_stream_upload( s ) ) return st;
  HIP_TRY( hipStreamSynchronize( s->ctx->copy ) );
  aa_dev_frame job;
  HIP_TRY( hipMemcpy( &job, r.dev_job, sizeof job, hipMemcpyDeviceToHost ) );
  if ( coeff_out && coeff_capacity_blocks < r.hdr.num_coeff_blocks ) return fail( AA_ERR_ARGUMENT, "aa_stream_read_records: coefficient buffer too small" );
  if ( !r.chunk_list ) {
    if ( mb_out ) HIP_TRY( hipMemcpy( mb_out, job.mbs, size_t( r.hdr.num_macroblocks ) * sizeof( aa_mb_info ), hipMemcpyDeviceToHost ) );
    if ( coeff_out ) HIP_TRY( hipMemcpy( coeff_out, job.coeffs, size_t( r.hdr.num_coeff_blocks ) * 32, hipMemcpyDeviceToHost ) );
    return AA_OK;
  }
  std::vector<aa_mb_info> mbs( r.hdr.num_macroblocks );
  HIP_TRY( hipMemcpy( mbs.data(), job.mbs, mbs.size() * sizeof( aa_mb_info ), hipMemcpyDeviceToHost ) );
  std::vector<uint32_t> list( size_t( r.est_chunks ) + 1 );
  HIP_TRY( hipMemcpy( list.data(), r.chunk_list, list.size() * sizeof( uint32_t ), hipMemcpyDeviceToHost ) );
  if ( list[0] != r.est_chunks ) return fail( AA_ERR_LOGIC, "aa_stream_read_records: chunk list disagrees with the parse summary" );
  if ( r.packed_pos ) {
    std::vector<uint32_t> pos( r.hdr.num_macroblocks );
    HIP_TRY( hipMemcpy( pos.data(), r.packed_pos, pos.size() * sizeof( uint32_t ), hipMemcpyDeviceToHost ) );
    std::vector<std::vector<int16_t>> words( list[0] );
    if ( coeff_out )
      for ( uint32_t k = 0; k < list[0]; k++ ) {
        words[k].resize( aa::kChunkWords );
        HIP_TRY( hipMemcpy( words[k].data(), s->ctx->tok.heap + size_t( list[1 + k] ) * kChunkBytesHeap, kChunkBytesHeap, hipMemcpyDeviceToHost ) );
      }
    uint32_t running = 0;
    for ( size_t mi = 0; mi < mbs.size(); mi++ ) {
      aa_mb_info & mb = mbs[mi];
      const uint32_t nblk = aa::pack::blocks_of( mb.nz_mask );
      if ( nblk && coeff_out ) {
        const uint32_t ord = pos[mi] >> 15, off = pos[mi] & ( aa::kChunkWords - 1u );
        if ( ord >= list[0] || running + nblk > r.hdr.num_coeff_blocks )
          return fail( AA_ERR_LOGIC, "aa_stream_read_records: a macroblock's coefficients lie outside the frame's chunks" );
        const int16_t * w = words[ord].data() + off, * end = words[ord].data() + aa::kChunkWords;
        if ( w + aa::pack::kMaskSlots > end ) return fail( AA_ERR_LOGIC, "aa_stream_read_records: packed coefficients run past their chunk" );
        uint32_t values = 0;
        for ( uint32_t b = 0; b < 25; b++ ) if ( ( mb.nz_mask >> b ) & 1u ) values += aa::pack::popc( static_cast<uint16_t>( w[b] ) );
        if ( w + aa::pack::kMaskSlots + values > end ) return fail( AA_ERR_LOGIC, "aa_stream_read_records: packed coefficients run past their chunk" );
        if ( ( static_cast<unsigned long long>( mb.reserved ) << 32 | mb.coeff_index ) != static_cast<unsigned long long>( list[1 + ord] ) * aa::kChunkWords + off )
          return fail( AA_ERR_LOGIC, "aa_stream_read_records: a macroblock's word offset disagrees with its place in the frame's chunks" );
        aa::pack::expand_macroblock( w, mb.nz_mask, coeff_out + size_t( running ) * 16 );
      }
      mb.coeff_index = running; mb.reserved = 0;
      running += nblk;
    }
    if ( running != r.hdr.num_coeff_blocks ) return fail( AA_ERR_LOGIC, "aa_stream_read_records: non-zero masks disagree with the parse summary" );
    if ( mb_out ) std::memcpy( mb_out, mbs.data(), mbs.size() * sizeof( aa_mb_info ) );
    return AA_OK;
  }
  std::map<uint32_t, std::vector<uint8_t>> chunk;
  if ( coeff_out )
    for ( uint32_t k = 0; k < list[0]; k++ ) {
      auto & v = chunk[list[1 + k]];
      v.resize( kChunkBytesHeap );
      HIP_TRY( hipMemcpy( v.data(), s->ctx->tok.heap + size_t( list[1 + k] ) * kChunkBytesHeap, kChunkBytesHeap, hipMemcpyDeviceToHost ) );
    }
  uint32_t running = 0;
  for ( auto & mb : mbs ) {
    const uint32_t nblk = static_cast<uint32_t>( __builtin_popcount( mb.nz_mask ) );
    if ( nblk && coeff_out ) {
      auto it = chunk.find( mb.coeff_index / aa::kChunkBlocks );
      if ( it == chunk.end() || mb.coeff_index % aa::kChunkBlocks + nblk > aa::kChunkBlocks || running + nblk > r.hdr.num_coeff_blocks )
        return fail( AA_ERR_LOGIC, "aa_stream_read_records: a macroblock's coefficients lie outside the frame's chunks" );
      std::memcpy( coeff_out + size_t( running ) * 16, it->second.data() + size_t( mb.coeff_index % aa::kChunkBlocks ) * 32, size_t( nblk ) * 32 );
    }
    mb.coeff_index = running;
    running += nblk;
  }
  if ( running != r.hdr.num_coeff_blocks ) return fail( AA_ERR_LOGIC, "aa_stream_read_records: non-zero masks disagree with the parse summary" );
  if ( mb_out ) std::memcpy( mb_out, mbs.data(), mbs.size() * sizeof( aa_mb_info ) );
  return AA_OK;
}

namespace {
aa_status launch_lf_rows( aa_ctx * ctx, std::vector<std::pair<uint32_t, const aa_dev_frame *>> & keyed, bool same_geometry, int max_mbh, int max_mbw )
{
  if ( !same_geometry ) std::stable_sort( keyed.begin(), keyed.end(), []( const auto & a, const auto & b ) { return a.first < b.first; } );
  aa_frame_list list;
  int filled = 0;
  auto launch = [&]() -> aa_status {
    if ( !filled ) return AA_OK;
    for ( int k = filled; k < AA_MAX_BATCH; k++ ) list.f[k] = nullptr;
    if ( aa_status st = zero_ws( ctx, ctx->ws, filled / 4, max_mbh ) ) return st;
    const size_t need = size_t( filled ) * max_mbh * max_mbw * 128;
    if ( need > ctx->boundary_bytes ) {
      HIP_TRY( hipStreamSynchronize( ctx->compute ) );
      if ( ctx->boundary ) (void) hipFree( ctx->boundary );
      ctx->boundary = nullptr; ctx->boundary_bytes = 0;
      HIP_TRY( hipMalloc( reinterpret_cast<void **>( &ctx->boundary ), need ) );
      ctx->boundary_bytes = need;
    }
    LaunchTimer t( ctx, 2 );
    if ( const int e = aa::launch_loopfilter_rows4( list, filled / 4, max_mbh, max_mbw, ctx->ws, ctx->boundary, ctx->n_xcd, ctx->compute ) ) return hip_fail( static_cast<hipError_t>( e ), "k_loopfilter_rows4" );
    filled = 0;
    return AA_OK;
  };
  for ( size_t i = 0; i < keyed.size(); ) {
    size_t j = i;
    while ( j < keyed.size() && j - i < 4 && keyed[j].first == keyed[i].first ) j++;
    for ( size_t k = 0; k < 4; k++ ) list.f[filled++] = i + k < j ? keyed[i + k].second : nullptr;
    i = j;
    if ( filled + 4 > AA_MAX_BATCH ) if ( aa_status st = launch() ) return st;
  }
  return launch();
}
}

namespace {
struct DecodeTiming {
  bool on = false; double ms[10] = { 0, 0, 0, 0, 0, 0, 0, 0, 0, 0 }; uint64_t calls = 0;
  ~DecodeTiming()
  {
    if ( !on || !calls ) return;
    static const char * const names[10] = { "checks", "stream uploads", "collect_pending", "resolve_summary (waits for the parser included)", "dense buffer",
                                            "bind_batch (waits for a binding buffer included)", "expand_packed", "job lists", "inter launches", "intra + loop-filter launches" };
    std::fprintf( stderr, "alfalfa_amd: aa_decode_batch host time over %llu calls, ms per call:", static_cast<unsigned long long>( calls ) );
    for ( int k = 0; k < 10; k++ ) std::fprintf( stderr, " [%s] %.3f", names[k], ms[k] / static_cast<double>( calls ) );
    std::fprintf( stderr, "\n" );
  }
};
DecodeTiming * decode_timing() { static DecodeTiming d; static const bool init = [] { const char * e = std::getenv( "ALFALFA_AMD_DECODE_TIMING" ); d.on = e && atoi( e ) != 0; return true; }(); (void) init; return &d; }
struct DecodeMark {
  DecodeTiming & d; double t;
  DecodeMark() : d( *decode_timing() ), t( d.on ? now_ms() : 0.0 ) { if ( d.on ) d.calls++; }
  void lap( int k ) { if ( d.on ) { const double n = now_ms(); d.ms[k] += n - t; t = n; } }
};
}

aa_status aa_decode_batch( aa_ctx * ctx, aa_stream * const * streams, int n, const int * frame_index )
{
  if ( !ctx || !streams || !frame_index || n <= 0 ) return fail( AA_ERR_ARGUMENT, "aa_decode_batch: bad argument" );
  if ( aa_status st = set_device( ctx ) ) return st;
  std::vector<const aa_dev_frame *> inter_jobs, intra_jobs, lf_jobs;
  std::vector<const FrameRec *> intra_recs;
  std::vector<uint32_t> lf_geometry;
  unsigned max_mbs = 0; int max_mbw = 0, max_mbh = 0;
  bool any_split = false;
  bool same_geometry = true;
  uint64_t total_mbs = 0;
  DecodeMark mk;
  for ( int i = 0; i < n; i++ ) {
    aa_stream * s = streams[i];
    if ( !s || s->ctx != ctx ) return fail( AA_ERR_ARGUMENT, "aa_decode_batch: stream belongs to another context" );
    const int fi = frame_index[i];
    if ( fi < 0 || fi >= static_cast<int>( s->frames.size() ) ) return fail( AA_ERR_ARGUMENT, "aa_decode_batch: frame index out of range" );
    if ( fi != s->next_submit ) return fail( AA_ERR_LOGIC, "aa_decode_batch: frames of a stream must be submitted in order" );
  }
  mk.lap( 0 );
  for ( int i = 0; i < n; i++ ) if ( aa_status st = aa_stream_upload( streams[i] ) ) return st;
  mk.lap( 1 );
  { std::lock_guard<std::mutex> g( ctx->pool_mu ); collect_pending( ctx, false ); }
  mk.lap( 2 );
  for ( int i = 0; i < n; i++ ) {
    if ( streams[i]->frames[frame_index[i]].records_released ) return fail( AA_ERR_LOGIC, "aa_decode_batch: frame records were released" );
    if ( aa_status st = resolve_summary( streams[i], streams[i]->frames[frame_index[i]] ) ) return st;
  }
  mk.lap( 3 );
  struct BindGuard { aa_ctx * c;
                     explicit BindGuard( aa_ctx * x ) : c( x ) { std::lock_guard<std::mutex> g( c->pool_mu ); c->binding_depth++; }
                     ~BindGuard() {
                       std::lock_guard<std::mutex> g( c->pool_mu );
                       if ( --c->binding_depth == 0 ) {
                         for ( auto & h : c->compute_hold ) { c->compute_free[h.second].push_back( h.first ); c->compute_free_bytes += h.second; }
                         c->compute_hold.clear();
                       } } } bind_guard( ctx );
  mk.lap( 4 );
  if ( aa_status st = bind_batch( ctx, streams, n, frame_index ) ) return st;
  mk.lap( 5 );
  struct Advance { aa_stream * const * streams; int n; bool ok = false; ~Advance() { if ( ok ) for ( int i = 0; i < n; i++ ) streams[i]->next_submit++; } } advance { streams, n };
  mk.lap( 6 );
  for ( int i = 0; i < n; i++ ) {
    aa_stream * s = streams[i];
    const FrameRec & r = s->frames[frame_index[i]];
    const aa_frame_header & h = r.hdr;
    if ( h.num_intra_mbs < h.num_macroblocks ) { inter_jobs.push_back( r.dev_job ); any_split = any_split || r.has_split; }
    if ( h.has_intra_mb ) { intra_jobs.push_back( r.dev_job ); intra_recs.push_back( &r ); }
    if ( h.loop_filter_level ) { lf_jobs.push_back( r.dev_job ); lf_geometry.push_back( ( static_cast<uint32_t>( h.mb_width ) << 16 ) | h.mb_height ); }
    if ( i > 0 && ( h.mb_width != streams[0]->frames[frame_index[0]].hdr.mb_width || h.mb_height != streams[0]->frames[frame_index[0]].hdr.mb_height ) ) same_geometry = false;
    max_mbs = std::max<unsigned>( max_mbs, h.num_macroblocks );
    max_mbw = std::max<int>( max_mbw, h.mb_width ); max_mbh = std::max<int>( max_mbh, h.mb_height );
    total_mbs += h.num_macroblocks;
  }
  ctx->stats.macroblocks += total_mbs;
  mk.lap( 7 );

  auto for_each_list = [&]( const std::vector<const aa_dev_frame *> & jobs, auto && fn ) -> int {
    for ( size_t base = 0; base < jobs.size(); base += AA_MAX_BATCH ) {
      aa_frame_list list;
      const int cnt = static_cast<int>( std::min<size_t>( AA_MAX_BATCH, jobs.size() - base ) );
      for ( int k = 0; k < cnt; k++ ) list.f[k] = jobs[base + k];
      for ( int k = cnt; k < AA_MAX_BATCH; k++ ) list.f[k] = nullptr;
      if ( int e = fn( list, cnt ) ) return e;
    }
    return 0;
  };
  auto check = [&]( int e, const char * what ) -> aa_status {
    if ( e ) return hip_fail( static_cast<hipError_t>( e ), what );
    return AA_OK;
  };

  if ( !inter_jobs.empty() ) {
    int e = for_each_list( inter_jobs, [&]( const aa_frame_list & l, int cnt ) {
      LaunchTimer t( ctx, 0 ); return aa::launch_recon_inter4( l, cnt, max_mbs, ctx->compute ); } );
    if ( aa_status st = check( e, "k_recon_inter4" ) ) return st;
    if ( any_split ) {
      e = for_each_list( inter_jobs, [&]( const aa_frame_list & l, int cnt ) {
        LaunchTimer t( ctx, 5 ); return aa::launch_recon_inter( l, cnt, max_mbs, true, ctx->compute ); } );
      if ( aa_status st = check( e, "k_recon_inter" ) ) return st;
    }
  }
  mk.lap( 8 );
  const int ndiag = max_mbw + 2 * ( max_mbh - 1 );
  if ( ctx->schedule == 0 ) {
    if ( aa_status st = ensure_ws( ctx, &ctx->ws, &ctx->ws_bytes, max_mbh ) ) return st;
    for ( size_t base = 0; base < intra_jobs.size(); base += AA_MAX_BATCH ) {
      aa_frame_list list;
      const int cnt = static_cast<int>( std::min<size_t>( AA_MAX_BATCH, intra_jobs.size() - base ) );
      const int groups = ( cnt + 3 ) / 4;
      for ( int k = 0; k < AA_MAX_BATCH; k++ ) list.f[k] = k < cnt ? intra_jobs[base + k] : nullptr;
      if ( aa_status st = zero_ws( ctx, ctx->ws, groups * 4, max_mbh ) ) return st;
      LaunchTimer t( ctx, 1 );
      if ( const int e = aa::launch_recon_intra4( list, groups, max_mbh, ctx->ws, ctx->n_xcd, ctx->compute ) ) return hip_fail( static_cast<hipError_t>( e ), "k_recon_intra4" );
    }
    if ( !lf_jobs.empty() ) {
      std::vector<std::pair<uint32_t, const aa_dev_frame *>> keyed;
      keyed.reserve( lf_geometry.size() );
      for ( size_t i = 0; i < lf_jobs.size(); i++ ) keyed.emplace_back( lf_geometry[i], lf_jobs[i] );
      if ( aa_status st = launch_lf_rows( ctx, keyed, same_geometry, max_mbh, max_mbw ) ) return st;
    }
    mk.lap( 9 );
    advance.ok = true;
    return AA_OK;
  }
  if ( !intra_jobs.empty() ) {
    for ( int d = 0; d < ndiag; d++ ) {
      bool needed = false;
      for ( const FrameRec * r : intra_recs ) if ( d < static_cast<int>( r->intra_diagonals.size() ) && r->intra_diagonals[d] ) { needed = true; break; }
      if ( !needed ) continue;
      const int row_lo = std::max( 0, ( d - ( max_mbw - 1 ) + 1 ) / 2 ), row_hi = std::min( max_mbh - 1, d / 2 );
      if ( row_hi < row_lo ) continue;
      const int e = for_each_list( intra_jobs, [&]( const aa_frame_list & l, int cnt ) {
        LaunchTimer t( ctx, 1 ); return aa::launch_recon_intra_diagonal( l, cnt, d, row_lo, row_hi - row_lo + 1, ctx->compute ); } );
      if ( aa_status st = check( e, "k_recon_intra" ) ) return st;
    }
  }
  if ( !lf_jobs.empty() ) {
    for ( int d = 0; d < ndiag; d++ ) {
      const int row_lo = std::max( 0, ( d - ( max_mbw - 1 ) + 1 ) / 2 ), row_hi = std::min( max_mbh - 1, d / 2 );
      if ( row_hi < row_lo ) continue;
      const int e = for_each_list( lf_jobs, [&]( const aa_frame_list & l, int cnt ) {
        LaunchTimer t( ctx, 2 ); return aa::launch_loopfilter_diagonal( l, cnt, d, row_lo, row_hi - row_lo + 1, ctx->compute ); } );
      if ( aa_status st = check( e, "k_loopfilter" ) ) return st;
    }
  }
  advance.ok = true;
  return AA_OK;
}

aa_status aa_stream_decode( aa_stream * s, const uint8_t * data, size_t size, int * frame_index, int * shown )
{
  int fi = -1; aa_frame_header h;
  if ( aa_status st = aa_stream_parse( s, data, size, &fi, &h ) ) return st;
  aa_stream * one[1] = { s };
  if ( aa_status st = aa_decode_batch( s->ctx, one, 1, &fi ) ) return st;
  if ( frame_index ) *frame_index = fi;
  if ( shown ) *shown = h.show_frame;
  return AA_OK;
}

int aa_stream_frame_count( const aa_stream * s ) { return s ? static_cast<int>( s->frames.size() ) : 0; }

aa_status aa_stream_set_error_concealment( aa_stream * s, int on )
{
  if ( !s ) return fail( AA_ERR_ARGUMENT, "null stream" );
  s->parser.set_error_concealment( on != 0 );
  return AA_OK;
}
int aa_stream_error_concealment( const aa_stream * s ) { return s && s->parser.error_concealment() ? 1 : 0; }

aa_status aa_stream_release_before( aa_stream * s, int first_kept )
{
  if ( !s ) return fail( AA_ERR_ARGUMENT, "null stream" );
  const int n = std::min<int>( first_kept, static_cast<int>( s->frames.size() ) );
  for ( int i = s->first_live; i < n; i++ ) {
    FrameRec & f = s->frames[i];
    if ( f.handle_held ) { f.handle_held = false; if ( f.placed ) release( s, f.out_slot ); }
// ... 29 lines not shown
```

### alfalfa_amd/csrc/runtime_submit.inc

```
namespace {
template <class Fill>
aa_status append_host_frame( aa_stream * s, int * frame_index, aa_frame_header * hdr_out, Fill && fill )
{
  if ( aa_status st = set_device( s->ctx ) ) return st;
  const size_t nmb = size_t( s->parser.mb_width() ) * s->parser.mb_height();
  const size_t job_bytes = align_up( sizeof( aa_dev_frame ) );
  const size_t mb_bytes = align_up( nmb * sizeof( aa_mb_info ) );
  const size_t words_per_row = ( s->parser.mb_width() + 63 ) / 64;
  const size_t rows_bytes = align_up( words_per_row * s->parser.mb_height() * sizeof( unsigned long long ) );
  const size_t worst = job_bytes + mb_bytes + rows_bytes + align_up( nmb * 25 * 32 );
  Chunk * c;
  if ( aa_status st = reserve( s, worst, &c ) ) return st;
  const size_t off = c->used;
  aa_dev_frame * job = reinterpret_cast<aa_dev_frame *>( c->host + off );
  aa_mb_info * mbs = reinterpret_cast<aa_mb_info *>( c->host + off + job_bytes );
  unsigned long long * intra_rows = reinterpret_cast<unsigned long long *>( c->host + off + job_bytes + mb_bytes );
  int16_t * coeffs = reinterpret_cast<int16_t *>( c->host + off + job_bytes + mb_bytes + rows_bytes );

  FrameRec rec;
  try { fill( rec.hdr, mbs, coeffs ); }
  catch ( const aa::ParseError & e ) { return fail( e.code, e.message ); }
  const aa_frame_header & h = rec.hdr;
  c->used = off + job_bytes + mb_bytes + rows_bytes + align_up( size_t( h.num_coeff_blocks ) * 32 );

  const int mbw = h.mb_width, mbh = h.mb_height;
  rec.intra_diagonals.assign( mbw + 2 * ( mbh - 1 ), 0 );
  std::memset( intra_rows, 0, words_per_row * mbh * sizeof( unsigned long long ) );
  if ( h.has_intra_mb )
    for ( int r = 0; r < mbh; r++ ) for ( int col = 0; col < mbw; col++ )
      if ( !( mbs[r * mbw + col].flags & AA_MB_INTER ) ) {
        rec.intra_diagonals[col + 2 * r] = 1;
        intra_rows[r * words_per_row + ( col >> 6 )] |= 1ull << ( col & 63 );
      }

  if ( !h.key_frame )
    for ( size_t i = 0; i < nmb; i++ ) if ( mbs[i].y_mode == 9  ) { rec.has_split = true; break; }

  fill_job( rec, job );
  job->mbs = reinterpret_cast<const aa_mb_info *>( c->dev + off + job_bytes );
  job->intra_rows = reinterpret_cast<const unsigned long long *>( c->dev + off + job_bytes + mb_bytes );
  job->coeffs = reinterpret_cast<const int16_t *>( c->dev + off + job_bytes + mb_bytes + rows_bytes );
  rec.host_job = job;
  rec.dev_job = reinterpret_cast<const aa_dev_frame *>( c->dev + off );
  rec.chunk = static_cast<int>( c - s->chunks.data() );
  c->live_frames++;
  const int fi = static_cast<int>( s->frames.size() );
  s->frames.push_back( std::move( rec ) );
  if ( frame_index ) *frame_index = fi;
  if ( hdr_out ) *hdr_out = h;
  return AA_OK;
}
}
extern "C" {

aa_status aa_stream_parse( aa_stream * s, const uint8_t * data, size_t size, int * frame_index, aa_frame_header * hdr_out )
{
  if ( !s || !data ) return fail( AA_ERR_ARGUMENT, "aa_stream_parse: null argument" );
  if ( aa_status st = set_device( s->ctx ) ) return st;
  if ( aa_status st = segmap_to_host( s ) ) return st;
  return append_host_frame( s, frame_index, hdr_out, [&]( aa_frame_header & hdr, aa_mb_info * mbs, int16_t * coeffs ) { s->parser.parse( data, size, hdr, mbs, coeffs ); } );
}

aa_status aa_stream_append_records( aa_stream * s, const aa_frame_header * hdr, const aa_mb_info * mbs_in, const int16_t * coeffs_in, int * frame_index )
{
  if ( !s || !hdr || !mbs_in ) return fail( AA_ERR_ARGUMENT, "aa_stream_append_records: null argument" );
  if ( hdr->num_coeff_blocks && !coeffs_in ) return fail( AA_ERR_ARGUMENT, "aa_stream_append_records: coefficient blocks missing" );
  const size_t nmb = size_t( s->parser.mb_width() ) * s->parser.mb_height();
  if ( hdr->mb_width != s->parser.mb_width() || hdr->mb_height != s->parser.mb_height() || hdr->num_macroblocks != nmb )
    return fail( AA_ERR_ARGUMENT, "aa_stream_append_records: the header's macroblock dimensions are not this decoder's" );
  if ( hdr->num_coeff_blocks > nmb * 25 ) return fail( AA_ERR_ARGUMENT, "aa_stream_append_records: more coefficient blocks than macroblocks can hold" );
  uint32_t intra = 0;
  for ( size_t i = 0; i < nmb; i++ ) {
    const uint32_t nblk = static_cast<uint32_t>( __builtin_popcount( mbs_in[i].nz_mask & 0x1FFFFFFu ) );
    if ( ( mbs_in[i].nz_mask >> 25 ) || ( nblk && size_t( mbs_in[i].coeff_index ) + nblk > hdr->num_coeff_blocks ) )
      return fail( AA_ERR_ARGUMENT, "aa_stream_append_records: macroblock " + std::to_string( i ) + " points outside the coefficient blocks" );
    if ( mbs_in[i].y_mode > 9 || mbs_in[i].uv_mode > 3 || mbs_in[i].ref_frame > 3 || mbs_in[i].segment_id > 3 || mbs_in[i].lf_level > 63 )
      return fail( AA_ERR_ARGUMENT, "aa_stream_append_records: macroblock " + std::to_string( i ) + " has a field out of range" );
    if ( !( mbs_in[i].flags & AA_MB_INTER ) ) intra++;
    else if ( hdr->key_frame ) return fail( AA_ERR_ARGUMENT, "aa_stream_append_records: inter macroblock in a key frame" );
  }
  return append_host_frame( s, frame_index, nullptr, [&]( aa_frame_header & h, aa_mb_info * mbs, int16_t * coeffs ) {
    h = *hdr;
    h.num_intra_mbs = intra; h.has_intra_mb = intra != 0;
    std::memcpy( mbs, mbs_in, nmb * sizeof( aa_mb_info ) );
    if ( hdr->num_coeff_blocks ) std::memcpy( coeffs, coeffs_in, size_t( hdr->num_coeff_blocks ) * 32 );
  } );
}

aa_status aa_stream_upload( aa_stream * s )
{
  if ( !s ) return fail( AA_ERR_ARGUMENT, "null stream" );
  if ( aa_status st = set_device( s->ctx ) ) return st;
  bool any = false;
  for ( auto & c : s->chunks ) {
    if ( c.host && c.uploaded < c.used ) {
      HIP_TRY( hipMemcpyAsync( c.dev + c.uploaded, c.host + c.uploaded, c.used - c.uploaded, hipMemcpyHostToDevice, s->ctx->copy ) );
      c.uploaded = c.used; any = true;
    }
  }
  if ( any ) {
    HIP_TRY( hipEventRecord( s->ctx->upload_done, s->ctx->copy ) );
    HIP_TRY( hipStreamWaitEvent( s->ctx->compute, s->ctx->upload_done, 0 ) );
  }
  return AA_OK;
}

aa_status aa_stream_release_staging( aa_stream * s )
{
  if ( !s ) return fail( AA_ERR_ARGUMENT, "null stream" );
  if ( aa_status st = set_device( s->ctx ) ) return st;
  if ( aa_status st = aa_stream_upload( s ) ) return st;
  HIP_TRY( hipStreamSynchronize( s->ctx->copy ) );
  for ( auto & c : s->chunks ) {
    if ( !c.host ) continue;
    { std::lock_guard<std::mutex> g( s->ctx->pool_mu ); s->ctx->pinned_pool.emplace_back( c.host, c.pinned_bytes ); }
    c.host = nullptr;
    c.capacity = c.used;
  }
  for ( auto & f : s->frames ) f.host_job = nullptr;
// ... 86 lines not shown
  }
  b->tokens_pending = false;
  ctx->deferred.erase( std::remove( ctx->deferred.begin(), ctx->deferred.end(), b ), ctx->deferred.end() );
  bool dropped = false;
  tok_prune_inflight( ctx );
  for ( int i = 0; i < b->n; i++ ) {
    Batch::Item & it = b->items[i];
    if ( !it.live ) { if ( jobs_host[i].nmb ) { jobs_host[i].nmb = 0; dropped = true; } continue; }
    FrameRec & r = it.s->frames[it.frame];
    if ( it.on_host ) continue;
    r.enqueued = true;
    if ( T.packed ) {
      const double words = std::min( double( aa::kMbWords ) * jobs_host[i].nmb, T.words_per_byte * 1.15 * jobs_host[i].size );
      r.est_chunks = static_cast<uint32_t>( words / ( aa::kChunkWords - aa::kMbWords ) ) + 1u;
    } else {
      const double blocks = std::min( 25.0 * jobs_host[i].nmb, T.blocks_per_byte * 1.15 * jobs_host[i].size );
      r.est_chunks = static_cast<uint32_t>( blocks / ( aa::kChunkBlocks - aa::kMbBlocks ) ) + 1u;
    }
    if ( T.lane_per_partition && jobs_host[i].mp_stride && jobs_host[i].fp.nparts > 1 ) r.est_chunks += static_cast<uint32_t>( jobs_host[i].fp.nparts ) - 1u;
    T.chunks_committed += r.est_chunks;
    ctx->stats.parsed_macroblocks += jobs_host[i].nmb;
  }
  if ( std::find( T.inflight.begin(), T.inflight.end(), b ) == T.inflight.end() ) T.inflight.push_back( b );
  if ( std::find( T.batches.begin(), T.batches.end(), b ) == T.batches.end() ) T.batches.push_back( b );
  if ( aa_status st = tok_grow_heap( ctx, static_cast<size_t>( std::max<int64_t>( 0, T.chunks_committed ) ) * kChunkBytesHeap ) ) return st;
  hipStream_t ps = b->ps;
  if ( b->patch_jobs && dropped ) HIP_TRY( hipMemcpyAsync( b->dev, b->host, b->head_bytes, hipMemcpyHostToDevice, ps ) );
  if ( dropped ) {
    int keep = 0;
    for ( int k = 0; k < b->n_order; k++ ) if ( b->items[b->launch_order_host[k]].live ) b->launch_order_host[keep++] = b->launch_order_host[k];
    b->n_order = keep;
    if ( keep ) HIP_TRY( hipMemcpyAsync( const_cast<uint32_t *>( b->launch_order_dev ), b->launch_order_host, size_t( keep ) * sizeof( uint32_t ), hipMemcpyHostToDevice, ps ) );
  }
  if ( b->n_order > 0 ) {
    if ( int e = aa::launch_enqueue_jobs( T.q, T.slots, reinterpret_cast<const aa::ParseJob *>( b->dev ), b->launch_order_dev, b->n_order, ps ) )
      return hip_fail( static_cast<hipError_t>( e ), "k_enqueue_jobs" );
    T.jobs_enqueued += static_cast<uint64_t>( b->n_order );
  }
  HIP_TRY( hipEventRecord( b->hdr_done, ps ) );
  HIP_TRY( hipEventRecord( ctx->parse_idle[b->parse_stream_index], ps ) );
  return tok_service( ctx, b->hdr_done );
}
}

namespace {
struct HostLaneScratch {
  uint8_t * pin = nullptr; size_t pin_bytes = 0;
  std::vector<uint8_t> above; hipEvent_t ev = nullptr;
  bool fit( size_t bytes )
  {
    if ( bytes <= pin_bytes ) return true;
    if ( pin ) (void) hipHostFree( pin );
    pin = nullptr; pin_bytes = 0;
    if ( hipHostMalloc( reinterpret_cast<void **>( &pin ), bytes, hipHostMallocDefault ) != hipSuccess ) { (void) hipGetLastError(); pin = nullptr; return false; }
    pin_bytes = bytes;
    return true;
  }
};
void host_lane_run( aa_ctx * ctx, Batch * b, int item, HostLaneScratch & S )
{
  const aa::ParseJob & J = reinterpret_cast<const aa::ParseJob *>( b->host )[item];
  volatile aa::FrameSummary * sum = reinterpret_cast<volatile aa::FrameSummary *>( b->host + b->summaries_off ) + item;
  Batch::Item & it = b->items[item];
  const uint32_t mbw = J.fp.mbw, mbh = J.fp.mbh, nmb = mbw * mbh;
  const size_t words_per_row = ( mbw + 63 ) / 64;
  uint32_t status = aa::TOK_OK, blocks = 0, intra = 0, split = 0;
  hipStream_t up = ctx->tok.host_up;
  if ( !S.ev ) status = aa::TOK_HOST_FAILED;
  const size_t mbs_bytes = align_up( size_t( nmb ) * sizeof( aa_mb_info ) ), rows_bytes = align_up( words_per_row * mbh * sizeof( unsigned long long ) );
  try { S.above.resize( size_t( mbw ) * 9 ); } catch ( const std::bad_alloc & ) { status = aa::TOK_HOST_FAILED; }
  if ( status == aa::TOK_OK && !S.fit( mbs_bytes + rows_bytes + size_t( nmb ) * 25 * 32 + 256 ) ) status = aa::TOK_HOST_FAILED;
  if ( status == aa::TOK_OK ) {
    aa_mb_info * mbs = reinterpret_cast<aa_mb_info *>( S.pin );
    unsigned long long * rows = reinterpret_cast<unsigned long long *>( S.pin + mbs_bytes );
    int16_t * coeffs = reinterpret_cast<int16_t *>( S.pin + mbs_bytes + rows_bytes );
    std::memset( static_cast<void *>( mbs ), 0, size_t( nmb ) * sizeof( aa_mb_info ) );
    const double t_parse = now_ms();
    aa::parse_frame_body( b->host + it.data_off, J.fp, mbs, coeffs, S.above.data(), &blocks, &intra );
    ctx->host_lanes.parse_us += static_cast<uint64_t>( ( now_ms() - t_parse ) * 1e3 ); ctx->host_lanes.parsed_bytes += J.size;
    std::memset( rows, 0, words_per_row * mbh * sizeof( unsigned long long ) );
    for ( uint32_t r = 0; r < mbh; r++ ) for ( uint32_t c = 0; c < mbw; c++ ) {
      const aa_mb_info & mb = mbs[r * mbw + c];
      if ( !( mb.flags & AA_MB_INTER ) ) rows[r * words_per_row + ( c >> 6 )] |= 1ull << ( c & 63 );
      else if ( mb.y_mode == aa::SPLITMV ) split = 1;
    }
    uint8_t * dense = nullptr;
    const size_t dense_bytes = align_up( std::max<size_t>( size_t( blocks ) * 32, 32 ) );
    hipError_t e = hipSuccess;
    if ( dev_alloc( ctx, dense_bytes, &dense ) != AA_OK ) status = aa::TOK_HOST_FAILED;
    else {
      it.host_dense = dense; it.host_dense_bytes = dense_bytes;
      e = hipMemcpyAsync( J.mbs, mbs, size_t( nmb ) * sizeof( aa_mb_info ), hipMemcpyHostToDevice, up );
      if ( e == hipSuccess ) e = hipMemcpyAsync( J.intra_rows, rows, words_per_row * mbh * sizeof( unsigned long long ), hipMemcpyHostToDevice, up );
      if ( e == hipSuccess && blocks ) e = hipMemcpyAsync( dense, coeffs, size_t( blocks ) * 32, hipMemcpyHostToDevice, up );
      if ( e == hipSuccess ) {
        uint8_t * job_dev = b->dev + align_up( size_t( b->n ) * sizeof( aa::ParseJob ) ) + size_t( item ) * sizeof( aa_dev_frame );
        const int16_t ** dense_ptr = reinterpret_cast<const int16_t **>( S.pin + S.pin_bytes - 16 );
        *dense_ptr = reinterpret_cast<const int16_t *>( dense );
        e = hipMemcpyAsync( job_dev + offsetof( aa_dev_frame, coeffs ), dense_ptr, sizeof *dense_ptr, hipMemcpyHostToDevice, up );
      }
      if ( e == hipSuccess ) e = hipEventRecord( S.ev, up );
      if ( e == hipSuccess ) e = hipEventSynchronize( S.ev );
      if ( e != hipSuccess ) status = aa::TOK_HOST_FAILED;
    }
  }
  sum->num_coeff_blocks = blocks; sum->num_intra_mbs = intra; sum->has_split = split; sum->steps = 0; sum->num_chunks = 0; sum->packed_words = 0;
  sum->status = status;
  ctx->host_lanes.backlog_bytes -= J.size;
  __atomic_thread_fence( __ATOMIC_RELEASE );
  sum->done = 1u;
}
void host_lanes_main( aa_ctx * ctx )
{
  (void) hipSetDevice( ctx->device );
  HostLaneScratch S;
  for ( int tries = 0; tries < 3 && !S.ev; tries++ )
    if ( hipEventCreateWithFlags( &S.ev, hipEventDisableTiming ) != hipSuccess ) { (void) hipGetLastError(); S.ev = nullptr; usleep( 1000 ); }
  auto & H = ctx->host_lanes;
  for ( ;; ) {
    aa_ctx::HostLanes::Task t;
    {
      std::unique_lock<std::mutex> g( H.mu );
      H.cv.wait( g, [&] { return H.stop || !H.q.empty(); } );
      if ( H.q.empty() ) break;
      t = H.q.front(); H.q.pop_front();
    }
    host_lane_run( ctx, t.b, t.item, S );
  }
  if ( S.ev ) (void) hipEventDestroy( S.ev );
  if ( S.pin ) (void) hipHostFree( S.pin );
}
void host_lanes_start( aa_ctx * ctx )
{
  auto & H = ctx->host_lanes;
  if ( !H.threads.empty() ) return;
  int nt = effective_cpus();
  if ( const char * e = std::getenv( "ALFALFA_AMD_HOST_LANES" ) ) nt = std::max( 1, atoi( e ) );
  for ( int t = 0; t < nt; t++ ) H.threads.emplace_back( host_lanes_main, ctx );
}
double host_lanes_rate( aa_ctx * ctx )
{
  auto & H = ctx->host_lanes;
  int nt = static_cast<int>( H.threads.size() );
  if ( !nt ) { nt = effective_cpus(); if ( const char * e = std::getenv( "ALFALFA_AMD_HOST_LANES" ) ) nt = std::max( 1, atoi( e ) ); }
  const uint64_t us = H.parse_us.load(), bytes = H.parsed_bytes.load();
  const double per_worker = us > 1000 ? static_cast<double>( bytes ) / static_cast<double>( us ) * 1e3 : 24.0e3;
  return per_worker * std::min( nt, effective_cpus() );
}
void host_lanes_stop( aa_ctx * ctx )
{
  auto & H = ctx->host_lanes;
  { std::lock_guard<std::mutex> g( H.mu ); H.stop = true; }
  H.cv.notify_all();
  for ( auto & t : H.threads ) t.join();
  H.threads.clear();
}
}

aa_status aa_launch_tokens( aa_ctx * ctx, int max_batches, int * launched_out )
{
  if ( !ctx ) return fail( AA_ERR_ARGUMENT, "aa_launch_tokens: null context" );
  if ( aa_status st = set_device( ctx ) ) return st;
  int launched = 0;
  while ( !ctx->deferred.empty() && ( max_batches <= 0 || launched < max_batches ) ) {
    if ( aa_status st = launch_tokens_of( ctx, ctx->deferred.front() ) ) return st;
    launched++;
  }
// ... 278 lines not shown
```

### alfalfa_amd/csrc/runtime_types.inc

```
namespace {

thread_local std::string g_last_error;


aa_status fail( aa_status code, const std::string & msg ) { g_last_error = msg; return code; }

int effective_cpus()
{
  static const int n = [] {
    int cpus = static_cast<int>( std::thread::hardware_concurrency() );
    if ( cpus < 1 ) cpus = 1;
    cpu_set_t set;
    if ( sched_getaffinity( 0, sizeof set, &set ) == 0 ) { const int a = CPU_COUNT( &set ); if ( a > 0 && a < cpus ) cpus = a; }
    auto read_two = []( const char * path, double * a, double * b ) -> int {
      FILE * f = std::fopen( path, "r" );
      if ( !f ) return 0;
      char first[64] = { 0 };
      int got = std::fscanf( f, "%63s %lf", first, b );
      std::fclose( f );
      if ( got < 1 ) return 0;
      if ( std::strcmp( first, "max" ) == 0 ) { *a = -1; return got; }
      *a = atof( first );
      return got;
    };
    double quota = -1, period = 100000;
    if ( read_two( "/sys/fs/cgroup/cpu.max", &quota, &period ) < 1 ) {
      double q = -1, dummy = 0;
      if ( read_two( "/sys/fs/cgroup/cpu/cpu.cfs_quota_us", &q, &dummy ) >= 1 ) { quota = q; double pp = 100000; if ( read_two( "/sys/fs/cgroup/cpu/cpu.cfs_period_us", &pp, &dummy ) >= 1 && pp > 0 ) period = pp; }
    }
    if ( quota > 0 && period > 0 ) { const int q = std::max( 1, static_cast<int>( quota / period + 0.5 ) ); if ( q < cpus ) cpus = q; }
    return cpus;
  }();
  return n;
}
int worker_threads( int asked )
{
  const int cap = std::max( 1, std::min( 256, 2 * effective_cpus() ) );
  return std::max( 1, std::min( asked > 0 ? asked : cap, cap ) );
}
aa_status hip_fail( hipError_t e, const char * what )
{
  return fail( e == hipErrorNoDevice || e == hipErrorInvalidDevice ? AA_ERR_NO_DEVICE : AA_ERR_HIP,
               std::string( what ) + ": " + hipGetErrorString( e ) );
}
#define HIP_TRY( expr ) do { hipError_t e__ = ( expr ); if ( e__ != hipSuccess ) return hip_fail( e__, #expr ); } while ( 0 )

constexpr size_t kChunkBytes = size_t( 64 ) << 20;
constexpr size_t kAlign = 256;
inline size_t align_up( size_t v, size_t a = kAlign ) { return ( v + a - 1 ) / a * a; }

struct Chunk {
  uint8_t * host = nullptr;
  uint8_t * dev = nullptr;
  size_t capacity = 0, used = 0, uploaded = 0;
  size_t pinned_bytes = 0;
  size_t dev_bytes = 0;
  int live_frames = 0;
};

struct Batch {
  uint8_t * host = nullptr, * dev = nullptr;
  size_t host_bytes = 0, dev_bytes = 0;
  int n = 0, live = 0;
  hipEvent_t hdr_done = nullptr;
  size_t summaries_off = 0;
  uint8_t * host_dev = nullptr;
  bool tokens_pending = false;
  bool patch_jobs = false;
  size_t head_bytes = 0;
  const uint32_t * launch_order_dev = nullptr;
  uint32_t * launch_order_host = nullptr;
  int n_order = 0;
  int max_mbw = 0, max_nparts = 1;
  hipStream_t ps = nullptr;
  int parse_stream_index = 0;
  struct Item { aa_stream * s; int frame; bool live; bool on_host = false; size_t data_off = 0; uint8_t * host_dense = nullptr; size_t host_dense_bytes = 0; };
  std::vector<Item> items;
};

struct Slot {
  uint8_t * dev = nullptr;
  bool shared = false;
  int refs = 0;
  bool hash_valid = false;
  uint64_t hash = 0;
};

struct FrameRec {
  aa_frame_header hdr;
  aa_dev_frame * host_job = nullptr;
  const aa_dev_frame * dev_job = nullptr;
  int out_slot = -1;
  int ref_after[3] = { -1, -1, -1 };
  std::vector<uint8_t> intra_diagonals;
  bool has_split = false;
  bool handle_held = true;
  int chunk = -1;
  Batch * batch = nullptr;
  int batch_item = -1;
  bool summary_pending = false;
  uint8_t * rec_block = nullptr;
  size_t rec_bytes = 0;
  bool rec_in_arena = false;
  const uint32_t * chunk_list = nullptr;
  aa_mb_info * dev_mbs = nullptr;
  const uint32_t * packed_pos = nullptr;
  volatile aa::FrameSummary * summary = nullptr;
  const aa::ParseJob * parse_job = nullptr;
  bool enqueued = false;
  uint32_t est_chunks = 0;
  bool chunks_returned = false;
  bool records_released = false;
  bool placed = false;
};

}

struct aa_parser { aa::Parser impl; aa_parser( uint16_t w, uint16_t h ) : impl( w, h ) {} };

struct aa_ctx {
  int device = 0;
  hipStream_t compute = nullptr, copy = nullptr;
  hipEvent_t upload_done = nullptr;
  std::atomic<int> refs { 1 };
  struct BindBuf { aa_raster_binding * host = nullptr, * dev = nullptr; size_t cap = 0; hipEvent_t done = nullptr; bool busy = false; };
  static constexpr int kBindBufs = 16;
  BindBuf bind_bufs[kBindBufs];
  int next_bind_buf = 0;
  struct HostLanes {
    struct Task { Batch * b; int item; };
    std::mutex mu; std::condition_variable cv;
    std::deque<Task> q;
    std::vector<std::thread> threads;
    bool stop = false;
    std::atomic<uint64_t> parsed_bytes { 0 }, parse_us { 0 }, backlog_bytes { 0 };
    uint64_t parse_us_mark = 0;
  } host_lanes;
  struct GatherBuf { aa_gather_job * host = nullptr, * dev = nullptr; size_t cap = 0; hipEvent_t done = nullptr, copied = nullptr; bool busy = false; };
  GatherBuf gather_bufs[kBindBufs];
  int next_gather_buf = 0;
  struct RgbBuf { uint8_t * host = nullptr, * dev = nullptr; size_t cap = 0; hipEvent_t done = nullptr, before = nullptr, after = nullptr; bool busy = false; };
  RgbBuf rgb_bufs[kBindBufs];
  int next_rgb_buf = 0;
  RgbBuf quality_bufs[kBindBufs];
  int next_quality_buf = 0;
  int row_handoff_by_kernel[2] = { 0, 0 };
  std::deque<int> downloads_in_flight;
  static constexpr int kMaxParseStreams = 20;
  int n_parse_streams = 4;
  std::vector<hipStream_t> parse_streams;
  std::vector<hipEvent_t> parse_idle;
  int prio_low = 0;
  int next_parse_stream = 0;
  hipEvent_t last_seg_batch = nullptr;
  std::vector<Batch *> deferred;
  struct Tok {
    bool ready = false;
    hipStream_t util = nullptr;
    hipStream_t host_up = nullptr;
    aa::TokQueue * q = nullptr;
    unsigned long long * slots = nullptr;
    uint32_t q_slots = 1u << 18;
    uint64_t jobs_enqueued = 0;
    std::vector<Batch *> inflight;
    std::vector<Batch *> batches;
    uint32_t * one_dev = nullptr;
    uint8_t * heap = nullptr;
    size_t heap_va = 0, heap_mapped = 0, heap_limit = 0, grow_bytes = size_t( 1 ) << 30;
    bool vmm = false;
    std::vector<hipMemGenericAllocationHandle_t> handles;
    aa::CoeffPool * pool = nullptr;
    uint32_t * ring = nullptr;
    int64_t chunks_committed = 0;
    double blocks_per_byte = 1.0;
    bool packed = true;
    bool lane_per_partition = false;
    uint32_t mp_hint = 1;
    double words_per_byte = 4.0;
// ... 82 lines not shown
```

### alfalfa_amd/csrc/tok_fsm.hh

```
#pragma once
#include <initializer_list>

#include "parse_common.hh"

namespace aa {

struct alignas( 16 ) V16 { uint32_t x, y, z, w; };
struct alignas( 8 ) V8 { uint32_t x, y; };

#if defined( __HIP_DEVICE_COMPILE__ )
#define AA_GLOBAL __attribute__( ( address_space( 1 ) ) )
#else
#define AA_GLOBAL
#endif

struct FrameSummary {
  uint32_t num_coeff_blocks;
  uint32_t num_intra_mbs;
  uint32_t has_split;
  uint32_t steps;
  uint32_t num_chunks;
  uint32_t status;
  uint32_t done;
  uint32_t packed_words;
};
enum : uint32_t { TOK_OK = 0, TOK_STEP_BOUND = 1, TOK_NO_MEMORY = 2,
                  TOK_HOST_FAILED = 3 };

#if defined( __HIP_DEVICE_COMPILE__ )
#define AA_AT_ADD( p, v ) __hip_atomic_fetch_add( ( p ), ( v ), __ATOMIC_RELAXED, __HIP_MEMORY_SCOPE_AGENT )
#define AA_AT_ADD_ACQ( p, v ) __hip_atomic_fetch_add( ( p ), ( v ), __ATOMIC_ACQUIRE, __HIP_MEMORY_SCOPE_AGENT )
#define AA_AT_ADD_REL( p, v ) __hip_atomic_fetch_add( ( p ), ( v ), __ATOMIC_RELEASE, __HIP_MEMORY_SCOPE_AGENT )
#define AA_AT_LOAD( p ) __hip_atomic_load( ( p ), __ATOMIC_RELAXED, __HIP_MEMORY_SCOPE_AGENT )
#define AA_AT_STORE( p, v ) __hip_atomic_store( ( p ), ( v ), __ATOMIC_RELAXED, __HIP_MEMORY_SCOPE_AGENT )
#define AA_NOW() wall_clock64()
#else
template <class T, class V> AA_HD inline T aa_host_add( T * p, V v ) { const T old = *p; *p = static_cast<T>( old + static_cast<T>( v ) ); return old; }
#define AA_AT_ADD( p, v ) aa::aa_host_add( ( p ), ( v ) )
#define AA_AT_ADD_ACQ( p, v ) aa::aa_host_add( ( p ), ( v ) )
#define AA_AT_ADD_REL( p, v ) aa::aa_host_add( ( p ), ( v ) )
#define AA_AT_LOAD( p ) ( *( p ) )
#define AA_AT_STORE( p, v ) ( *( p ) = ( v ) )
AA_HD inline unsigned long long aa_host_clock() { static unsigned long long t = 0; return t += 1000; }
#define AA_NOW() aa::aa_host_clock()
#endif

struct CoeffPool {
  int32_t avail;
  uint32_t head;
  uint32_t reserve, publish;
  uint32_t mask;
  uint32_t starving;
  uint32_t pad[2];
};
constexpr uint32_t kChunkBlocks = 2048;
constexpr uint32_t kNoChunk = 0xFFFFFFFFu;
constexpr uint32_t kMbBlocks = 26;
constexpr uint32_t kChunkWords = kChunkBlocks * 16u;
constexpr uint32_t kMbMaskSlots = 25u;
constexpr uint32_t kMbWords = kMbMaskSlots + 25u * 16u;
AA_HD constexpr uint32_t chunk_list_entries( uint32_t nmb, uint32_t lanes = 1 ) { return 2u + ( nmb + 75u ) / 76u + 2u * ( lanes - 1u ); }

struct TokQueue {
  uint32_t head, reserve, publish, mask;
};

struct Heap {
  AA_GLOBAL int16_t * base;
  AA_GLOBAL CoeffPool * pool;
  AA_GLOBAL uint32_t * ring;
};

struct alignas( 16 ) ParseJob {
  FrameParams fp;
  const uint8_t * data;
  uint32_t size, data_padded;
  uint32_t nmb, flags_padded;
  aa_mb_info * mbs;
  uint32_t * chunk_list;
  uint32_t mp_stride;
  uint32_t mp_pad;
  uint32_t * packed_pos;
  unsigned long long * intra_rows;
  uint8_t * mbflags;
  FrameSummary * summary;
};

AA_HD inline uint32_t mp_flag_index( const ParseJob & J, uint32_t row, uint32_t col )
{
  const uint32_t P = J.fp.nparts;
  return J.flags_padded + ( row % P ) * J.mp_stride + ( row / P ) * J.fp.mbw + col;
}
AA_HD constexpr uint32_t mp_flag_stride( uint32_t mbw, uint32_t mbh, uint32_t P ) { return ( ( ( mbh + P - 1u ) / P ) * mbw + 15u ) & ~15u; }

namespace tok {

constexpr uint32_t kPeriod = 32;
constexpr uint32_t kRing = 128;
constexpr uint32_t kChunks = 2;
constexpr uint32_t kMetaRing = 32;
constexpr uint32_t kMetaChunks = 1;
static_assert( kRing >= 3 * kPeriod && 16 * kChunks == kPeriod && ( kRing & ( kRing - 1 ) ) == 0, "stream ring invariant" );

constexpr uint32_t kNodeTabOff = 0;
constexpr uint32_t kBandTabOff = 384;
constexpr uint32_t kXtab = 408;
constexpr uint32_t kSignX = 26;
constexpr uint32_t kBlockTabOff = 440;
// ... 816 lines not shown
```

### alfalfa_amd/decoder.py

```python
import collections
import ctypes as C
import struct

import numpy as np

from . import capi
from .capi import AlfalfaError, FrameHeader, MB_INFO_DTYPE


Quality = collections.namedtuple("Quality", ["ssim", "sse"])


class Parser:

    def __init__(self, width, height):
        self.L = capi.lib()
        self.h = C.c_void_p()
        capi.check(self.L.aa_parser_create(width, height, C.byref(self.h)))
        self.width, self.height = width, height
        self.mbw, self.mbh = (width + 15) // 16, (height + 15) // 16
        n = self.mbw * self.mbh
        self._mb = np.zeros(n, dtype=MB_INFO_DTYPE)
        self._coeff = np.zeros(n * 25 * 16, dtype=np.int16)

# ... 269 lines not shown
        compute = None
        if not cur.cuda_stream:
            compute = torch.cuda.ExternalStream(self.compute_stream(), device=device)
            compute.wait_stream(cur)
        capi.check(self.L.aa_quality_batch_async(self.h, arr, n, idx, refs, np_, C.c_void_p(ssim.data_ptr()), C.c_void_p(sse.data_ptr()),
                                                 C.c_void_p(cur.cuda_stream or None)))
        if compute is not None:
            cur.wait_stream(compute)
        return Quality(ssim, sse)

    def decode_batch(self, decoders, frame_indices):
        n = len(decoders)
        arr = (C.c_void_p * n)(*[d.h for d in decoders])
        idx = (C.c_int * n)(*frame_indices)
        capi.check(self.L.aa_decode_batch(self.h, arr, n, idx))


class Decoder:

    def __init__(self, ctx, width, height):
        self.ctx, self.L = ctx, capi.lib()
        self.h = C.c_void_p()
        capi.check(self.L.aa_stream_create(ctx.h, width, height, C.byref(self.h)))
        self.width, self.height = width, height
        self.padded_width, self.padded_height = capi.raster_geometry(width, height)

    def __del__(self):
        if getattr(self, "h", None):
            self.L.aa_stream_destroy(self.h); self.h = None

    def set_error_concealment(self, on):
        capi.check(self.L.aa_stream_set_error_concealment(self.h, int(on)))

    def error_concealment(self):
        return bool(self.L.aa_stream_error_concealment(self.h))

    def parse_frame(self, frame_bytes):
        fi, hdr = C.c_int(), FrameHeader()
        capi.check(self.L.aa_stream_parse(self.h, frame_bytes, len(frame_bytes), C.byref(fi), C.byref(hdr)))
        return fi.value, hdr.as_dict()

    def append_records(self, header, mb, coeff_blocks):
        hdr = FrameHeader()
        for n, _ in FrameHeader._fields_:
            if n == "quant":
                for sgm in range(4):
                    for k in range(6):
                        hdr.quant[sgm][k] = header["quant"][sgm][k]
            else:
                setattr(hdr, n, header[n])
        mbs = np.ascontiguousarray(mb, dtype=MB_INFO_DTYPE).reshape(-1)
        cf = np.ascontiguousarray(coeff_blocks, dtype=np.int16).reshape(-1, 16)
        hdr.num_coeff_blocks = len(cf)
        fi = C.c_int()
        capi.check(self.L.aa_stream_append_records(self.h, C.byref(hdr), mbs.ctypes.data_as(C.c_void_p), cf.ctypes.data_as(C.c_void_p), C.byref(fi)))
        return fi.value

    def upload(self):
        capi.check(self.L.aa_stream_upload(self.h))

    def release_staging(self):
        capi.check(self.L.aa_stream_release_staging(self.h))

    def decode_frame(self, frame_index):
        self.ctx.decode_batch([self], [frame_index])

    def get_frame_output(self, frame_bytes):
        fi, shown = C.c_int(), C.c_int()
        capi.check(self.L.aa_stream_decode(self.h, frame_bytes, len(frame_bytes), C.byref(fi), C.byref(shown)))
        return bool(shown.value), fi.value

    def parse_and_decode_frame(self, frame_bytes):
        shown, fi = self.get_frame_output(frame_bytes)
        return fi if shown else None

    def frame_count(self):
        return self.L.aa_stream_frame_count(self.h)

    def frame_header(self, frame_index):
        hdr = FrameHeader()
        capi.check(self.L.aa_stream_frame_header(self.h, frame_index, C.byref(hdr)))
        return hdr.as_dict()

    def read_records(self, frame_index):
        h = self.frame_header(frame_index)
        mbw, mbh = h["mb_width"], h["mb_height"]
        mb = np.zeros(mbw * mbh, dtype=MB_INFO_DTYPE)
        cf = np.zeros((max(1, h["num_coeff_blocks"]), 16), dtype=np.int16)
        capi.check(self.L.aa_stream_read_records(self.h, frame_index, mb.ctypes.data_as(C.c_void_p), cf.ctypes.data_as(C.c_void_p), len(cf)))
        return h, mb.reshape(mbh, mbw), cf[:h["num_coeff_blocks"]]

    def rewind(self):
        capi.check(self.L.aa_stream_rewind(self.h))

    def decoder_hash(self):
        parts, whole = (C.c_uint64 * 4)(), C.c_uint64()
        capi.check(self.L.aa_stream_decoder_hash(self.h, parts, C.byref(whole)))
        return list(parts), whole.value

    def minihash(self):
        h = C.c_uint32()
        capi.check(self.L.aa_stream_minihash(self.h, C.byref(h)))
        return h.value

    def raster_hash(self, frame_index):
        h = C.c_uint64()
        capi.check(self.L.aa_stream_raster_hash(self.h, frame_index, C.byref(h)))
        return h.value

    def release_frame(self, frame_index):
        capi.check(self.L.aa_stream_release_frame(self.h, frame_index))

    def rewind_to(self, frame_index):
        capi.check(self.L.aa_stream_rewind_to(self.h, frame_index))

    def lf_search(self, frame_bytes, original_luma, level_lo, level_hi, want_rasters=False):
        n = level_hi - level_lo + 1
        orig = np.ascontiguousarray(original_luma, dtype=np.uint8)
        assert orig.shape == (self.padded_height, self.padded_width), orig.shape
        best, q = C.c_int(), C.c_double()
        qs = (C.c_double * n)()
        rb = sum(self.plane_sizes())
        rasters = np.empty(n * rb, np.uint8) if want_rasters else None
        capi.check(self.L.aa_stream_lf_search(self.h, frame_bytes, len(frame_bytes), orig.ctypes.data_as(C.c_void_p), level_lo, level_hi,
                                              C.byref(best), C.byref(q), qs, rasters.ctypes.data_as(C.c_void_p) if want_rasters else None))
        return best.value, q.value, list(qs), ([rasters[i * rb:(i + 1) * rb].tobytes() for i in range(n)] if want_rasters else None)

    def release_before(self, first_kept):
        capi.check(self.L.aa_stream_release_before(self.h, first_kept))

    def raster(self, frame_index):
        pw, ph = self.padded_width, self.padded_height
        y = np.empty((ph, pw), np.uint8); u = np.empty((ph // 2, pw // 2), np.uint8); v = np.empty((ph // 2, pw // 2), np.uint8)
        capi.check(self.L.aa_stream_download(self.h, frame_index, y.ctypes.data_as(C.c_void_p), u.ctypes.data_as(C.c_void_p), v.ctypes.data_as(C.c_void_p)))
        return y, u, v

    def download_async(self, frame_index, y_ptr, u_ptr, v_ptr):
        capi.check(self.L.aa_stream_download_async(self.h, frame_index, C.c_void_p(y_ptr), C.c_void_p(u_ptr), C.c_void_p(v_ptr)))

    def download_wait(self):
        capi.check(self.L.aa_stream_download_wait(self.h))

    def raster_bytes(self, frame_index):
        return b"".join(p.tobytes() for p in self.raster(frame_index))

    def display_bytes(self, frame_index):
        y, u, v = self.raster(frame_index)
        w, h = self.width, self.height
        return y[:h, :w].tobytes() + u[:(h + 1) // 2, :(w + 1) // 2].tobytes() + v[:(h + 1) // 2, :(w + 1) // 2].tobytes()

    def rgb(self, frame_index, format="rgb24", mean=None, std=None, out=None):
        return self.ctx.to_rgb([self], [frame_index], format, mean, std, None if out is None else [out])[0]

    def quality(self, frame_index, original, planes="y"):
        q = self.ctx.quality([self], [frame_index], [original], planes)
        return Quality(q.ssim[0], q.sse[0])

    def raster_device_pointers(self, frame_index):
        y, u, v = C.c_void_p(), C.c_void_p(), C.c_void_p()
        capi.check(self.L.aa_stream_raster_device(self.h, frame_index, C.byref(y), C.byref(u), C.byref(v)))
        return y.value, u.value, v.value

    def get_references(self):
        a, b, c = C.c_int(), C.c_int(), C.c_int()
        capi.check(self.L.aa_stream_references(self.h, C.byref(a), C.byref(b), C.byref(c)))
        return {"last": a.value, "golden": b.value, "alternative": c.value}

    def export_state(self):
        n = self.L.aa_stream_state_size(self.h)
        buf = (C.c_uint8 * n)()
        capi.check(self.L.aa_stream_export_state(self.h, buf, n))
        return bytes(buf)

    def import_state(self, blob):
        capi.check(self.L.aa_stream_import_state(self.h, blob, len(blob)))

    def serialize(self):
        n = C.c_size_t(0)
        capi.check(self.L.aa_stream_serialize(self.h, None, 0, C.byref(n)))
        buf = (C.c_uint8 * n.value)()
        capi.check(self.L.aa_stream_serialize(self.h, buf, n.value, C.byref(n)))
        return bytes(buf)

    def deserialize(self, blob):
        capi.check(self.L.aa_stream_deserialize(self.h, blob, len(blob)))

    def plane_sizes(self):
        pw, ph = self.padded_width, self.padded_height
        return pw * ph, (pw // 2) * (ph // 2), (pw // 2) * (ph // 2)

    def export_raster_device(self, frame_index, y_ptr, u_ptr, v_ptr):
        capi.check(self.L.aa_stream_export_raster(self.h, frame_index, C.c_void_p(y_ptr), C.c_void_p(u_ptr), C.c_void_p(v_ptr)))

    def import_reference_device(self, y_ptr, u_ptr, v_ptr):
        capi.check(self.L.aa_stream_import_reference(self.h, C.c_void_p(y_ptr), C.c_void_p(u_ptr), C.c_void_p(v_ptr)))

    def import_reference_host(self, y, u, v):
        y, u, v = (np.ascontiguousarray(p, dtype=np.uint8) for p in (y, u, v))
        capi.check(self.L.aa_stream_import_reference_host(self.h, y.ctypes.data_as(C.c_void_p), u.ctypes.data_as(C.c_void_p), v.ctypes.data_as(C.c_void_p)))


def psnr(sse, width, height, planes):
    import torch
    pixels = [float(width * height)] + [float((width // 2) * (height // 2))] * 2
    count = torch.tensor(pixels[:Context.QUALITY_PLANES[planes]], dtype=torch.float64, device=sse.device)
    s = sse.to(torch.float64)
    return torch.where(s == 0, torch.full_like(s, float("inf")), 10.0 * torch.log10(255.0 * 255.0 * count / s))


def read_ivf(path_or_bytes):
    data = path_or_bytes if isinstance(path_or_bytes, (bytes, bytearray)) else open(path_or_bytes, "rb").read()
    if data[:4] != b"DKIF":
        raise AlfalfaError(-1, "invalid bitstream: missing IVF file header")
    if struct.unpack_from("<H", data, 4)[0] != 0:
        raise AlfalfaError(-2, "unsupported bitstream: not an IVF version 0 file")
    hdr_len = struct.unpack_from("<H", data, 6)[0]
    if hdr_len != 32:
        raise AlfalfaError(-2, "unsupported bitstream: unsupported IVF header length")
    width, height = struct.unpack_from("<HH", data, 12)
    nframes = struct.unpack_from("<I", data, 24)[0]
    frames, pos = [], hdr_len
    for _ in range(nframes):
        if pos + 12 > len(data):
            raise AlfalfaError(-1, "invalid bitstream: IVF file truncated")
        n = struct.unpack_from("<I", data, pos)[0]
        if pos + 12 + n > len(data):
            raise AlfalfaError(-1, "invalid bitstream: IVF file truncated")
        frames.append(bytes(data[pos + 12:pos + 12 + n])); pos += 12 + n
    return width, height, frames


class FilePlayer:

    def __init__(self, ctx, path_or_bytes):
        self.width, self.height, self.frames = read_ivf(path_or_bytes)
        self.decoder = Decoder(ctx, self.width, self.height)
        self.frame_no = 0
        while self.frame_no < len(self.frames) and (self.frames[self.frame_no][0] & 1):
            self.frame_no += 1

    def eof(self):
        return self.frame_no == len(self.frames)

    def advance(self):
        while not self.eof():
            fi = self.decoder.parse_and_decode_frame(self.frames[self.frame_no]); self.frame_no += 1
            if fi is not None:
                return fi
        raise AlfalfaError(-2, "unsupported bitstream: hidden frames at end of file")
```

### include/alfalfa_amd.h

```cpp
#ifndef ALFALFA_AMD_H
#define ALFALFA_AMD_H

#include <stddef.h>
#include <stdint.h>

#ifdef __cplusplus
extern "C" {
#endif

#define AA_ABI_VERSION 4

typedef enum aa_status {
  AA_OK = 0,
  AA_ERR_INVALID = -1,
  AA_ERR_UNSUPPORTED = -2,
  AA_ERR_LOGIC = -3,
  AA_ERR_OUT_OF_RANGE = -4,
  AA_ERR_HIP = -5,
  AA_ERR_NO_DEVICE = -6,
  AA_ERR_ARGUMENT = -7,
  AA_ERR_NO_MEMORY = -8
} aa_status;

const char * aa_last_error( void );
// ... 54 lines not shown
aa_status aa_parser_parse( aa_parser * p, const uint8_t * data, size_t size,
                           aa_frame_header * hdr_out, aa_mb_info * mb_out, int16_t * coeff_out );

aa_status aa_parser_set_error_concealment( aa_parser * p, int on );
aa_status aa_parse_frame_tag( const uint8_t * data, size_t size, uint16_t width, uint16_t height, int accept_partial,
                              int * key_frame, int * show_frame, int * experimental, int * corruption_level );

aa_status aa_parser_get_probs( const aa_parser * p, uint8_t probs[1101] );
aa_status aa_parser_get_segmentation( const aa_parser * p, int * enabled, int * absolute, int8_t quant[4], int8_t lf[4], uint8_t * map );
aa_status aa_parser_get_filter_adjustments( const aa_parser * p, int * enabled, int8_t ref[4], int8_t mode[4] );

size_t aa_parser_state_size( const aa_parser * p );
aa_status aa_parser_export_state( const aa_parser * p, uint8_t * buf, size_t capacity );
aa_status aa_parser_import_state( aa_parser * p, const uint8_t * buf, size_t size );

aa_status aa_parser_serialize_state( const aa_parser * p, uint8_t * buf, size_t capacity, size_t * size );
aa_status aa_parser_deserialize_state( aa_parser * p, const uint8_t * buf, size_t size );

typedef struct aa_ctx aa_ctx;
typedef struct aa_stream aa_stream;

aa_status aa_ctx_create( int device, aa_ctx ** out );
void aa_ctx_destroy( aa_ctx * ctx );
aa_status aa_ctx_sync( aa_ctx * ctx );
aa_status aa_ctx_memory( aa_ctx * ctx, size_t * free_bytes, size_t * total_bytes );
#define AA_SCHEDULE_ROWS 0
#define AA_SCHEDULE_DIAGONAL 1
aa_status aa_ctx_set_schedule( aa_ctx * ctx, int schedule );
aa_status aa_ctx_clear_error( aa_ctx * ctx );
aa_status aa_ctx_set_memory_limit( aa_ctx * ctx, size_t bytes );
typedef struct aa_ctx_info {
  uint64_t memory_limit_bytes;
  uint64_t pool_bytes;
  uint64_t pool_free_bytes;
  uint64_t pool_pending_bytes;
  uint64_t heap_mapped_bytes;
  uint64_t heap_limit_bytes;
  uint64_t heap_used_bytes;
  uint64_t pinned_host_bytes;
  uint32_t heap_is_virtual;
  uint32_t token_lanes_per_workgroup, token_workgroups_capacity, token_workgroups_alive;
  uint32_t token_lane_lds_bytes, token_workgroup_lds_bytes;
  uint32_t jobs_waiting;
  uint32_t compute_units;
  int32_t heap_free_chunks;
  uint32_t lanes_starved;
  uint64_t token_profile[8];
  uint32_t packed_coefficients;
  uint32_t lane_per_partition;
  uint32_t clock_mhz;
  uint32_t host_share_ms;
  uint32_t host_rate_kb_per_ms;
  uint32_t reserved1;
  uint32_t stream_concurrency;
  uint32_t streams_needed;
  uint32_t host_waited_parse_ms;
  uint32_t host_waited_compute_ms;
} aa_ctx_info;
aa_status aa_ctx_get_info( aa_ctx * ctx, aa_ctx_info * out );
aa_status aa_ctx_set_packed_coefficients( aa_ctx * ctx, int on );
aa_status aa_ctx_set_host_share_ms( aa_ctx * ctx, double ms );
aa_status aa_ctx_set_lane_per_partition( aa_ctx * ctx, int on );
void * aa_ctx_compute_stream( aa_ctx * ctx );
void * aa_ctx_copy_stream( aa_ctx * ctx );

aa_status aa_stream_create( aa_ctx * ctx, uint16_t width, uint16_t height, aa_stream ** out );
void aa_stream_destroy( aa_stream * s );

aa_status aa_stream_parse( aa_stream * s, const uint8_t * data, size_t size, int * frame_index, aa_frame_header * hdr_out );
aa_status aa_stream_append_records( aa_stream * s, const aa_frame_header * hdr, const aa_mb_info * mbs, const int16_t * coeffs, int * frame_index );
aa_status aa_stream_upload( aa_stream * s );
aa_status aa_stream_release_staging( aa_stream * s );
aa_status aa_decode_batch( aa_ctx * ctx, aa_stream * const * streams, int n, const int * frame_index );
aa_status aa_stream_decode( aa_stream * s, const uint8_t * data, size_t size, int * frame_index, int * shown );

typedef struct aa_frame_in { aa_stream * stream; const uint8_t * data; size_t size; } aa_frame_in;
aa_status aa_submit_frames( aa_ctx * ctx, const aa_frame_in * frames, int n, int * frame_index_out, int threads );
#define AA_SUBMIT_DEFER_TOKENS 1u
#define AA_SUBMIT_DEVICE 2u
#define AA_SUBMIT_HOST 4u
aa_status aa_submit_frames_ex( aa_ctx * ctx, const aa_frame_in * frames, int n, int * frame_index_out, int threads, unsigned flags );
aa_status aa_launch_tokens( aa_ctx * ctx, int max_batches, int * launched_out );
aa_status aa_stream_frame_header( aa_stream * s, int frame_index, aa_frame_header * out );
aa_status aa_stream_read_records( aa_stream * s, int frame_index, aa_mb_info * mb_out, int16_t * coeff_out, size_t coeff_capacity_blocks );

aa_status aa_stream_set_error_concealment( aa_stream * s, int on );
int aa_stream_error_concealment( const aa_stream * s );

int aa_stream_frame_count( const aa_stream * s );
aa_status aa_stream_release_before( aa_stream * s, int first_kept );
aa_status aa_stream_rewind( aa_stream * s );
aa_status aa_stream_rewind_to( aa_stream * s, int frame_index );

aa_status aa_stream_download( aa_stream * s, int frame_index, uint8_t * y, uint8_t * u, uint8_t * v );
aa_status aa_pinned_alloc( aa_ctx * ctx, size_t bytes, void ** out );
void aa_pinned_free( void * p );
aa_status aa_stream_download_async( aa_stream * s, int frame_index, uint8_t * y, uint8_t * u, uint8_t * v );
aa_status aa_stream_download_wait( aa_stream * s );
aa_status aa_download_batch_async( aa_ctx * ctx, aa_stream * const * streams, int n, const int * frame_index, uint8_t * dst, size_t stride );
aa_status aa_ctx_download_wait( aa_ctx * ctx );
aa_status aa_ctx_download_wait_until( aa_ctx * ctx, int max_in_flight );
aa_status aa_stream_raster_device( aa_stream * s, int frame_index, void ** y, void ** u, void ** v );
enum { AA_RGB_U8_HWC3 = 0, AA_RGB_U8_HWC4 = 1, AA_RGB_U8_CHW = 2, AA_RGB_F16_CHW = 3, AA_RGB_BF16_CHW = 4, AA_RGB_F32_CHW = 5 };
typedef struct aa_rgb_target { void * dst; int64_t row_stride; int64_t plane_stride; } aa_rgb_target;
aa_status aa_render_rgb_async( aa_ctx * ctx, aa_stream * const * streams, int n, const int * frame_index, int format,
                               const aa_rgb_target * targets, const double mean[3], const double std[3], void * consumer_stream );
enum { AA_QUALITY_Y = 1, AA_QUALITY_YUV = 3 };
typedef struct aa_quality_ref { const void * y, * u, * v; int64_t y_stride, uv_stride; } aa_quality_ref;
aa_status aa_quality_batch_async( aa_ctx * ctx, aa_stream * const * streams, int n, const int * frame_index,
                                  const aa_quality_ref * originals, int planes,
                                  double * ssim_dev, uint64_t * sse_dev, void * consumer_stream );
aa_status aa_stream_references( const aa_stream * s, int * last, int * golden, int * alternate );
aa_status aa_stream_reference_slots( const aa_stream * s, int slots[3] );
aa_status aa_stream_import_reference( aa_stream * s, const void * y_dev, const void * u_dev, const void * v_dev );
aa_status aa_stream_import_reference_host( aa_stream * s, const uint8_t * y, const uint8_t * u, const uint8_t * v );

aa_status aa_stream_export_raster( aa_stream * s, int frame_index, void * y_dev, void * u_dev, void * v_dev );
size_t aa_stream_state_size( const aa_stream * s );
aa_status aa_stream_export_state( const aa_stream * s, uint8_t * buf, size_t capacity );
aa_status aa_stream_import_state( aa_stream * s, const uint8_t * buf, size_t size );

aa_status aa_stream_serialize( aa_stream * s, uint8_t * buf, size_t capacity, size_t * size );
aa_status aa_stream_deserialize( aa_stream * s, const uint8_t * buf, size_t size );

aa_status aa_parser_state_hash( const aa_parser * p, uint64_t * out );
aa_status aa_stream_state_hash( aa_stream * s, uint64_t * out );
aa_status aa_stream_raster_hash( aa_stream * s, int frame_index, uint64_t * out );
aa_status aa_stream_decoder_hash( aa_stream * s, uint64_t parts[4], uint64_t * whole );
aa_status aa_stream_minihash( aa_stream * s, uint32_t * out );
aa_status aa_stream_release_frame( aa_stream * s, int frame_index );
aa_status aa_stream_set_references( aa_stream * s, const void * const planes[3][3], const int is_host[3] );
aa_status aa_stream_reference_device( aa_stream * s, int which, void ** y, void ** u, void ** v );
aa_status aa_stream_reference_download( aa_stream * s, int which, uint8_t * y, uint8_t * u, uint8_t * v );

void aa_raster_geometry( uint16_t width, uint16_t height, uint32_t * padded_width, uint32_t * padded_height );

aa_status aa_stream_lf_search( aa_stream * s, const uint8_t * data, size_t size, const uint8_t * original_luma,
                               int level_lo, int level_hi, int * best_level, double * best_ssim, double * ssim_out, uint8_t * rasters_out );

aa_status aa_ssim_host( const uint8_t * a, const uint8_t * b, int width, int height, double * out );

typedef struct aa_kernel_stats {
  double recon_inter_ms, recon_intra_ms, loopfilter_ms;
  uint64_t recon_inter_launches, recon_intra_launches, loopfilter_launches;
  uint64_t macroblocks;
  double parse_headers_ms, parse_tokens_ms;
  uint64_t parse_launches;
  uint64_t parsed_macroblocks;
  double recon_split_ms;
  uint64_t recon_split_launches;
  uint64_t pool_waits;
  double pool_wait_ms, parse_wait_ms;
  double bind_wait_ms;
  double alloc_ms;
  uint64_t slab_mallocs;
  uint64_t token_steps;
  uint64_t token_frames;
  uint64_t worker_launches, worker_wgs;
  uint64_t worker_retires;
  uint64_t heap_grows;
  uint64_t heap_mapped_bytes;
  uint64_t nomem_retries;
  uint64_t frames_evicted;
  uint64_t host_routed_frames;
  uint64_t row_handoff_stale_polls;
  uint64_t row_handoff_rereads;
  uint64_t packed_frames, packed_words, packed_blocks;
  double host_batch_ms, host_batch_parse_wall_ms, host_batch_parse_cpu_ms, host_batch_arena_ms;
  uint64_t pinned_allocs;
} aa_kernel_stats;
aa_status aa_ctx_profile( aa_ctx * ctx, int enable );
aa_status aa_ctx_kernel_stats( aa_ctx * ctx, aa_kernel_stats * out, int reset );

#ifdef __cplusplus
}
#endif
#endif
```

Before: 126.6 million.

## Specialize inter recon for frames whose luma vectors are all full-pixel

The token parser and the host path now record per frame whether any non-split inter macroblock has a fractional luma motion vector. Frames without one are sent to a templated k_recon_inter4 variant that copies luma straight from the reference (vector loads when in bounds), skips the luma six-tap filtering, and uses a smaller LDS layout. Chroma still filters when needed and falls back to a byte-aligned copy otherwise. This adds a second launch per batch when frames of both kinds are mixed, plus a device error flag that catches a wrong summary.

```diff
diff --git a/alfalfa_amd/__init__.py b/alfalfa_amd/__init__.py
--- a/alfalfa_amd/__init__.py
+++ b/alfalfa_amd/__init__.py
@@ -2,4 +2,4 @@
 
 _os.environ.setdefault("GPU_MAX_HW_QUEUES", "16")
 
-from .decoder import AlfalfaError, Context, Decoder, FilePlayer, Parser, Quality, psnr, read_ivf
+from .decoder import AlfalfaError, Context, Decoder, FilePlayer, Parser, Quality, frame_marks_of_records, psnr, read_ivf
diff --git a/alfalfa_amd/capi.py b/alfalfa_amd/capi.py
--- a/alfalfa_amd/capi.py
+++ b/alfalfa_amd/capi.py
@@ -49,7 +49,7 @@
                 ("worker_retires", C.c_uint64), ("heap_grows", C.c_uint64), ("heap_mapped_bytes", C.c_uint64), ("nomem_retries", C.c_uint64), ("frames_evicted", C.c_uint64), ("host_routed_frames", C.c_uint64),
                 ("row_handoff_stale_polls", C.c_uint64), ("row_handoff_rereads", C.c_uint64), ("packed_frames", C.c_uint64), ("packed_words", C.c_uint64), ("packed_blocks", C.c_uint64),
                 ("host_batch_ms", C.c_double), ("host_batch_parse_wall_ms", C.c_double), ("host_batch_parse_cpu_ms", C.c_double), ("host_batch_arena_ms", C.c_double),
-                ("pinned_allocs", C.c_uint64)]
+                ("pinned_allocs", C.c_uint64), ("recon_inter_copy_launches", C.c_uint64), ("recon_inter_general_launches", C.c_uint64)]
 
 
 class CtxInfo(C.Structure):
@@ -118,6 +118,8 @@
     ("aa_stream_lf_search", C.c_int, [_P, C.c_char_p, C.c_size_t, C.c_void_p, C.c_int, C.c_int, C.POINTER(C.c_int), C.POINTER(C.c_double),
                                       C.POINTER(C.c_double), C.c_void_p]),
     ("aa_stream_frame_header", C.c_int, [_P, C.c_int, C.POINTER(FrameHeader)]),
+    ("aa_stream_frame_marks", C.c_int, [_P, C.c_int, C.POINTER(C.c_uint)]),
+    ("aa_frame_marks_of_records", C.c_uint, [_P, C.c_size_t]),
     ("aa_stream_read_records", C.c_int, [_P, C.c_int, _P, _P, C.c_size_t]),
     ("aa_stream_frame_count", C.c_int, [_P]), ("aa_stream_release_before", C.c_int, [_P, C.c_int]),
     ("aa_stream_rewind", C.c_int, [_P]), ("aa_stream_rewind_to", C.c_int, [_P, C.c_int]),
diff --git a/alfalfa_amd/csrc/device_types.h b/alfalfa_amd/csrc/device_types.h
--- a/alfalfa_amd/csrc/device_types.h
+++ b/alfalfa_amd/csrc/device_types.h
@@ -96,7 +96,7 @@
 int launch_pool_push_range( const Heap & heap, uint32_t first, uint32_t count, void * stream );
 int launch_pool_free_lists( const Heap & heap, const uint32_t * const * lists, int n, void * stream );
 int launch_mirror_counters( const TokQueue * q, const CoeffPool * pool, const uint32_t * exited, int n_grids, const unsigned long long * prof, aa_tok_mirror * out, uint32_t seq, void * stream );
-int launch_recon_inter4( const aa_frame_list & list, int n, unsigned max_mbs, void * stream );
+int launch_recon_inter4( const aa_frame_list & list, int n, unsigned max_mbs, bool luma_copy, aa_sync_ws * ws, void * stream );
 int launch_recon_inter( const aa_frame_list & list, int n, unsigned max_mbs, bool split_only, void * stream );
 int launch_recon_intra_diagonal( const aa_frame_list & list, int n, int diagonal, int row_lo, int rows, void * stream );
 int launch_loopfilter_diagonal( const aa_frame_list & list, int n, int diagonal, int row_lo, int rows, void * stream );
diff --git a/alfalfa_amd/csrc/kernels.hip b/alfalfa_amd/csrc/kernels.hip
--- a/alfalfa_amd/csrc/kernels.hip
+++ b/alfalfa_amd/csrc/kernels.hip
@@ -3,6 +3,7 @@
 #include <cstddef>
 
 #include <cstdlib>
+#include <type_traits>
 
 #include "device_types.h"
 #include "vp8_math.hh"
@@ -889,11 +890,31 @@
 };
 struct alignas( 16 ) Inter4Lds { Inter4Slot slot[4]; uint32_t taps[16]; };
 static_assert( offsetof( Inter4Slot, wc ) == offsetof( Inter4Slot, wy ) + 21 * 24, "wy and wc must be contiguous" );
-
-__device__ __forceinline__ void recon_inter4_body( const aa_dev_frame & f, const unsigned bq, const unsigned max_quads, Inter4Lds & L )
+struct alignas( 16 ) Inter4CopySlot {
+  alignas( 16 ) int16_t res[24][16];
+  union {
+    alignas( 16 ) uint8_t wc[2][13][16];
+    alignas( 16 ) uint8_t predc[128];
+  };
+  union {
+    alignas( 16 ) uint8_t tc[2][8][16];
+    alignas( 16 ) int16_t y2[32];
+  };
+};
+struct alignas( 16 ) Inter4CopyLds { Inter4CopySlot slot[4]; uint32_t taps[16]; };
+static_assert( sizeof( Inter4CopySlot::wc ) == 104 * 4 && offsetof( Inter4CopySlot, wc ) % 16 == 0, "wc is staged as 104 consecutive dwords" );
+static_assert( sizeof( Inter4CopySlot ) == 1440 && sizeof( Inter4CopyLds ) == 5824, "ten workgroups beside the token workers" );
+
+template <class T> __device__ __forceinline__ const __attribute__( ( address_space( 1 ) ) ) T * inter4_hbm( const void * p )
+{
+  return reinterpret_cast<const __attribute__( ( address_space( 1 ) ) ) T *>( reinterpret_cast<uintptr_t>( p ) );
+}
+
+template <bool kLumaCopy, class Lds>
+__device__ __forceinline__ void recon_inter4_body( const aa_dev_frame & f, const unsigned bq, const unsigned max_quads, Lds & L, int * const error )
 {
   const int lane = threadIdx.x, slot = lane >> 4, l = lane & 15;
-  Inter4Slot & S = L.slot[slot];
+  auto & S = L.slot[slot];
   if ( lane < 16 ) {
     uint32_t a, b; pack_taps( lane >> 1, a, b ); L.taps[lane] = ( lane & 1 ) ? b : a;
   }
@@ -919,6 +940,114 @@
   const int cmx = chroma_mv( 4 * mvx ), cmy = chroma_mv( 4 * mvy );
   const int sxy = col * 16 + ( mvx >> 3 ) - 2, syy = row * 16 + ( mvy >> 3 ) - 2;
   const int sxc = col * 8 + ( cmx >> 3 ) - 2, syc = row * 8 + ( cmy >> 3 ) - 2;
+  if constexpr ( kLumaCopy ) {
+    if ( __any( on && ( ( mvx | mvy ) & 7 ) != 0 ) ) { if ( lane == 0 ) atomicCAS( error, 0, 6 ); return; }
+    const int bx = col * 16 + ( mvx >> 3 ), by = row * 16 + ( mvy >> 3 );
+    const bool inside_y = bx >= 0 && by >= 0 && bx + 16 <= pw && by + 16 <= ph;
+    uint32_t py[4] = { 0, 0, 0, 0 };
+    if ( on && inside_y ) {
+      typedef uint32_t row16 __attribute__( ( ext_vector_type( 4 ), aligned( 1 ) ) );
+      const auto v = *inter4_hbm<row16>( ref_y + static_cast<ptrdiff_t>( by + l ) * pw + bx );
+      py[0] = v.x; py[1] = v.y; py[2] = v.z; py[3] = v.w;
+    } else if ( on ) {
+      const auto * const rp = inter4_hbm<uint8_t>( ref_y + static_cast<size_t>( clampi( by + l, 0, ph - 1 ) ) * pw );
+#pragma unroll
+      for ( int k = 0; k < 4; k++ )
+        py[k] = static_cast<uint32_t>( rp[clampi( bx + 4 * k, 0, pw - 1 )] ) | static_cast<uint32_t>( rp[clampi( bx + 4 * k + 1, 0, pw - 1 )] ) << 8
+              | static_cast<uint32_t>( rp[clampi( bx + 4 * k + 2, 0, pw - 1 )] ) << 16 | static_cast<uint32_t>( rp[clampi( bx + 4 * k + 3, 0, pw - 1 )] ) << 24;
+    }
+    const int axc = sxc & ~3;
+    const bool inside_c = sxc >= 0 && syc >= 0 && axc + 16 <= cw && syc + 13 <= ch;
+    const bool fast_c = on && inside_c;
+    uint32_t wreg[7];
+    const uint8_t * const wu0 = ref_u + static_cast<ptrdiff_t>( syc ) * cw + axc;
+    const uint8_t * const wv0 = ref_v + static_cast<ptrdiff_t>( syc ) * cw + axc;
+#pragma unroll
+    for ( int k = 0; k < 7; k++ ) {
+      const int i = l + 16 * k;
+      wreg[k] = 0;
+      if ( fast_c && i < 104 ) {
+        const int pl = i >= 52 ? 1 : 0, e = i - 52 * pl;
+        wreg[k] = *inter4_hbm<uint32_t>( ( pl ? wv0 : wu0 ) + static_cast<ptrdiff_t>( e >> 2 ) * cw + ( e & 3 ) * 4 );
+      }
+    }
+
+    residual_x4( S, f, has_res, has_y2, nz_mask, coeff_index, hd.y >> 24, segment, l );
+
+    {
+      uint32_t * flat = reinterpret_cast<uint32_t *>( &S.wc[0][0][0] );
+      if ( fast_c ) {
+#pragma unroll
+        for ( int k = 0; k < 7; k++ ) { const int i = l + 16 * k; if ( i < 104 ) flat[i] = wreg[k]; }
+      }
+      if ( on && !inside_c ) {
+        uint8_t * bc = &S.wc[0][0][0];
+        for ( int i = l; i < 2 * 13 * 16; i += 16 ) {
+          const int pl = i / 208, e = i % 208, r = e >> 4, c = e & 15;
+          bc[i] = ( pl ? ref_v : ref_u )[static_cast<size_t>( clampi( syc + r, 0, ch - 1 ) ) * cw + clampi( sxc + c, 0, cw - 1 )];
+        }
+      }
+    }
+    const int oc = inside_c ? ( sxc & 3 ) : 0;
+    __syncthreads();
+
+    const bool chroma_general = __any( on && ( ( cmx | cmy ) & 7 ) != 0 );
+    const uint8_t * const wcb = &S.wc[0][0][0]; uint8_t * const tcb = &S.tc[0][0][0];
+    uint2 copy_c = make_uint2( 0, 0 );
+    if ( chroma_general ) {
+      if ( on ) {
+        const int frac = cmx & 7;
+        const uint32_t t0 = L.taps[2 * frac], t1 = L.taps[2 * frac + 1];
+#pragma unroll
+        for ( int k = 0; k < 4; k++ ) {
+          const int j = l + 16 * k;
+          if ( k == 3 && j >= 52 ) continue;
+          const int pl = j >= 26 ? 1 : 0, e = j - 26 * pl, r = e >> 1, g = e & 1;
+          const uint8_t * sp = wcb + pl * 208 + r * 16 + g * 4;
+          const uint32_t o4 = sixtap_x4_lane( *reinterpret_cast<const uint32_t *>( sp ), *reinterpret_cast<const uint32_t *>( sp + 4 ), *reinterpret_cast<const uint32_t *>( sp + 8 ), oc, frac, t0, t1 );
+          uint8_t * tb = tcb + pl * 128 + ( g * 4 ) * 16 + r;
+          tb[0] = static_cast<uint8_t>( o4 ); tb[16] = static_cast<uint8_t>( o4 >> 8 ); tb[32] = static_cast<uint8_t>( o4 >> 16 ); tb[48] = static_cast<uint8_t>( o4 >> 24 );
+        }
+      }
+      __syncthreads();
+      if ( on ) {
+        const int frac = cmy & 7;
+        const uint32_t t0 = L.taps[2 * frac], t1 = L.taps[2 * frac + 1];
+#pragma unroll
+        for ( int k = 0; k < 2; k++ ) {
+          const int j = l + 16 * k, pl = j >> 4, c = ( j >> 1 ) & 7, i = j & 1;
+          const uint8_t * sp = tcb + pl * 128 + c * 16 + i * 4;
+          const uint32_t o4 = sixtap_x4_lane( *reinterpret_cast<const uint32_t *>( sp ), *reinterpret_cast<const uint32_t *>( sp + 4 ), *reinterpret_cast<const uint32_t *>( sp + 8 ), 0, frac, t0, t1 );
+          uint8_t * pb = S.predc + pl * 64 + ( i * 4 ) * 8 + c;
+          pb[0] = static_cast<uint8_t>( o4 ); pb[8] = static_cast<uint8_t>( o4 >> 8 ); pb[16] = static_cast<uint8_t>( o4 >> 16 ); pb[24] = static_cast<uint8_t>( o4 >> 24 );
+        }
+      }
+      __syncthreads();
+    } else if ( on ) {
+      const int pl = l >> 3, r = l & 7;
+      const uint2 * rp = reinterpret_cast<const uint2 *>( wcb + pl * 208 + ( r + 2 ) * 16 );
+      const uint2 a = rp[0], b = rp[1];
+      const bool q = oc + 2 >= 4; const int sft = ( oc + 2 ) & 3;
+      const uint32_t e0 = q ? a.y : a.x, e1 = q ? b.x : a.y, e2 = q ? b.y : b.x;
+      copy_c = make_uint2( __builtin_amdgcn_alignbyte( e1, e0, sft ), __builtin_amdgcn_alignbyte( e2, e1, sft ) );
+    }
+
+    if ( on ) {
+      uint32_t o[4];
+#pragma unroll
+      for ( int k = 0; k < 4; k++ ) o[k] = has_res ? add_residual_x4( py[k], &S.res[( l >> 2 ) * 4 + k][( l & 3 ) * 4] ) : py[k];
+      *reinterpret_cast<uint4 *>( f.cur[0] + static_cast<size_t>( row * 16 + l ) * pw + col * 16 ) = make_uint4( o[0], o[1], o[2], o[3] );
+      const int pl = l >> 3, r = l & 7;
+      uint32_t oc2[2];
+#pragma unroll
+      for ( int k = 0; k < 2; k++ ) {
+        const uint32_t p4 = chroma_general ? *reinterpret_cast<const uint32_t *>( S.predc + pl * 64 + r * 8 + 4 * k ) : ( k ? copy_c.y : copy_c.x );
+        oc2[k] = has_res ? add_residual_x4( p4, &S.res[16 + pl * 4 + ( r >> 2 ) * 2 + k][( r & 3 ) * 4] ) : p4;
+      }
+      *reinterpret_cast<uint2 *>( f.cur[1 + pl] + static_cast<size_t>( row * 8 + r ) * cw + col * 8 ) = make_uint2( oc2[0], oc2[1] );
+    }
+    return;
+  } else {
   const int axy = sxy & ~3, axc = sxc & ~3;
   const bool inside = sxy >= 0 && syy >= 0 && axy + 24 <= pw && syy + 21 <= ph && sxc >= 0 && syc >= 0 && axc + 16 <= cw && syc + 13 <= ch;
   const bool fast = on && inside;
@@ -1065,14 +1194,16 @@
     }
     *reinterpret_cast<uint2 *>( f.cur[1 + pl] + static_cast<size_t>( row * 8 + r ) * cw + col * 8 ) = make_uint2( oc2[0], oc2[1] );
   }
-}
-
-__global__ __launch_bounds__( kLanes ) void k_recon_inter4( const aa_frame_list list, const unsigned max_quads )
+  }
+}
+
+template <bool kLumaCopy>
+__global__ __launch_bounds__( kLanes ) void k_recon_inter4( const aa_frame_list list, const unsigned max_quads, int * const error )
 {
   __builtin_amdgcn_s_setprio( 3 );
 
-  __shared__ Inter4Lds L;
-  recon_inter4_body( *list.f[blockIdx.y], blockIdx.x, max_quads, L );
+  __shared__ std::conditional_t<kLumaCopy, Inter4CopyLds, Inter4Lds> L;
+  recon_inter4_body<kLumaCopy>( *list.f[blockIdx.y], blockIdx.x, max_quads, L, error );
 }
 
 constexpr int kStripMbs = 8;
@@ -1563,11 +1694,15 @@
   hipLaunchKernelGGL( k_recon_inter, dim3( blocks, n ), dim3( kLanes ), 0, static_cast<hipStream_t>( stream ), list, max_mbs, split_only ? 1 : 0 );
   return static_cast<int>( hipGetLastError() );
 }
-int launch_recon_inter4( const aa_frame_list & list, int n, unsigned max_mbs, void * stream )
+int launch_recon_inter4( const aa_frame_list & list, int n, unsigned max_mbs, bool luma_copy, aa_sync_ws * ws, void * stream )
 {
   const unsigned quads = ( max_mbs + 3u ) >> 2;
   const unsigned blocks = ( ( quads + 7u ) >> 3 ) * 8u;
-  hipLaunchKernelGGL( k_recon_inter4, dim3( blocks, n ), dim3( kLanes ), 0, static_cast<hipStream_t>( stream ), list, quads );
+  if ( luma_copy ) {
+    if ( !ws ) return static_cast<int>( hipErrorInvalidValue );
+    hipLaunchKernelGGL( k_recon_inter4<true>, dim3( blocks, n ), dim3( kLanes ), 0, static_cast<hipStream_t>( stream ), list, quads, &ws->error );
+  } else
+    hipLaunchKernelGGL( k_recon_inter4<false>, dim3( blocks, n ), dim3( kLanes ), 0, static_cast<hipStream_t>( stream ), list, quads, static_cast<int *>( nullptr ) );
   return static_cast<int>( hipGetLastError() );
 }
 int launch_recon_intra_diagonal( const aa_frame_list & list, int n, int diagonal, int row_lo, int rows, void * stream )
diff --git a/alfalfa_amd/csrc/parse_kernels.hip b/alfalfa_amd/csrc/parse_kernels.hip
--- a/alfalfa_amd/csrc/parse_kernels.hip
+++ b/alfalfa_amd/csrc/parse_kernels.hip
@@ -51,7 +51,8 @@
       J.mbflags[mi] = flags;
       if ( mp_stride ) J.mbflags[mp_row + col] = flags;
       if ( !( flags & AA_MB_INTER ) ) { intra++; word |= 1ull << ( col & 63 ); }
-      else if ( J.mbs[mi].y_mode == aa::SPLITMV ) split = 1;
+      else if ( J.mbs[mi].y_mode == aa::SPLITMV ) split |= aa::SUM_HAS_SPLIT;
+      else if ( ( J.mbs[mi].u.mv[0][0] | J.mbs[mi].u.mv[0][1] ) & 7 ) split |= aa::SUM_FRAC_LUMA;
       if ( ( col & 63 ) == 63 || col + 1 == mbw ) { J.intra_rows[row * words_per_row + ( col >> 6 )] = word; word = 0; }
     }
   }
diff --git a/alfalfa_amd/csrc/runtime_ctx.inc b/alfalfa_amd/csrc/runtime_ctx.inc
--- a/alfalfa_amd/csrc/runtime_ctx.inc
+++ b/alfalfa_amd/csrc/runtime_ctx.inc
@@ -221,6 +221,7 @@
   if ( !ctx->ws ) return AA_OK;
   int err = 0;
   HIP_TRY( hipMemcpy( &err, &ctx->ws->error, sizeof err, hipMemcpyDeviceToHost ) );
+  if ( err == 6 ) return fail( AA_ERR_HIP, "k_recon_inter4: the luma-copy variant met a luma vector with a fractional part: the frame's summary was wrong (output is not valid)" );
   if ( err == 3 ) return fail( AA_ERR_HIP, "row-pipelined kernel: a workgroup ran on an XCD outside the probed set (output is not valid)" );
   if ( err == 5 ) {
     int hdr[4] = {};
diff --git a/alfalfa_amd/csrc/runtime_decode.inc b/alfalfa_amd/csrc/runtime_decode.inc
--- a/alfalfa_amd/csrc/runtime_decode.inc
+++ b/alfalfa_amd/csrc/runtime_decode.inc
@@ -69,7 +69,8 @@
   r.hdr.num_coeff_blocks = sum->num_coeff_blocks;
   r.hdr.num_intra_mbs = sum->num_intra_mbs;
   r.hdr.has_intra_mb = sum->num_intra_mbs != 0;
-  r.has_split = sum->has_split != 0;
+  r.has_split = ( sum->has_split & aa::SUM_HAS_SPLIT ) != 0;
+  r.frac_luma = ( sum->has_split & aa::SUM_FRAC_LUMA ) != 0;
   r.intra_diagonals.assign( r.hdr.mb_width + 2 * ( r.hdr.mb_height - 1 ), r.hdr.has_intra_mb ? 1 : 0 );
   T.chunks_committed += static_cast<int64_t>( sum->num_chunks ) - static_cast<int64_t>( r.est_chunks );
   r.est_chunks = sum->num_chunks;
@@ -78,6 +79,23 @@
   if ( r.packed_pos ) { ctx->stats.packed_frames++; ctx->stats.packed_words += sum->packed_words; ctx->stats.packed_blocks += sum->num_coeff_blocks; }
   ctx->stats.token_steps += sum->steps; ctx->stats.token_frames++;
   r.summary_pending = false;
+  return AA_OK;
+}
+
+static_assert( AA_FRAME_HAS_SPLIT == aa::SUM_HAS_SPLIT && AA_FRAME_FRACTIONAL_LUMA == aa::SUM_FRAC_LUMA, "the public bits are the summary's" );
+unsigned aa_frame_marks_of_records( const aa_mb_info * mbs, size_t n )
+{
+  unsigned marks = 0;
+  for ( size_t i = 0; mbs && i < n; i++ ) marks |= aa::summary_marks_of( mbs[i] );
+  return marks;
+}
+
+aa_status aa_stream_frame_marks( aa_stream * s, int fi, unsigned * out )
+{
+  if ( !s || !out || fi < 0 || fi >= static_cast<int>( s->frames.size() ) ) return fail( AA_ERR_ARGUMENT, "aa_stream_frame_marks: bad argument" );
+  if ( aa_status st = set_device( s->ctx ) ) return st;
+  if ( aa_status st = resolve_summary( s, s->frames[fi] ) ) return st;
+  *out = ( s->frames[fi].has_split ? AA_FRAME_HAS_SPLIT : 0u ) | ( s->frames[fi].frac_luma ? AA_FRAME_FRACTIONAL_LUMA : 0u );
   return AA_OK;
 }
 
@@ -228,7 +246,7 @@
 {
   if ( !ctx || !streams || !frame_index || n <= 0 ) return fail( AA_ERR_ARGUMENT, "aa_decode_batch: bad argument" );
   if ( aa_status st = set_device( ctx ) ) return st;
-  std::vector<const aa_dev_frame *> inter_jobs, intra_jobs, lf_jobs;
+  std::vector<const aa_dev_frame *> inter_jobs, copy_jobs, general_jobs, intra_jobs, lf_jobs;
   std::vector<const FrameRec *> intra_recs;
   std::vector<uint32_t> lf_geometry;
   unsigned max_mbs = 0; int max_mbw = 0, max_mbh = 0;
@@ -270,7 +288,10 @@
     aa_stream * s = streams[i];
     const FrameRec & r = s->frames[frame_index[i]];
     const aa_frame_header & h = r.hdr;
-    if ( h.num_intra_mbs < h.num_macroblocks ) { inter_jobs.push_back( r.dev_job ); any_split = any_split || r.has_split; }
+    if ( h.num_intra_mbs < h.num_macroblocks ) {
+      inter_jobs.push_back( r.dev_job ); any_split = any_split || r.has_split;
+      ( r.frac_luma ? general_jobs : copy_jobs ).push_back( r.dev_job );
+    }
     if ( h.has_intra_mb ) { intra_jobs.push_back( r.dev_job ); intra_recs.push_back( &r ); }
     if ( h.loop_filter_level ) { lf_jobs.push_back( r.dev_job ); lf_geometry.push_back( ( static_cast<uint32_t>( h.mb_width ) << 16 ) | h.mb_height ); }
     if ( i > 0 && ( h.mb_width != streams[0]->frames[frame_index[0]].hdr.mb_width || h.mb_height != streams[0]->frames[frame_index[0]].hdr.mb_height ) ) same_geometry = false;
@@ -297,8 +318,15 @@
   };
 
   if ( !inter_jobs.empty() ) {
-    int e = for_each_list( inter_jobs, [&]( const aa_frame_list & l, int cnt ) {
-      LaunchTimer t( ctx, 0 ); return aa::launch_recon_inter4( l, cnt, max_mbs, ctx->compute ); } );
+    int e = 0;
+    if ( !copy_jobs.empty() ) {
+      if ( aa_status st = ensure_ws( ctx, &ctx->ws, &ctx->ws_bytes, max_mbh ) ) return st;
+      e = for_each_list( copy_jobs, [&]( const aa_frame_list & l, int cnt ) {
+        LaunchTimer t( ctx, 0 ); ctx->stats.recon_inter_copy_launches++; return aa::launch_recon_inter4( l, cnt, max_mbs, true, ctx->ws, ctx->compute ); } );
+      if ( aa_status st = check( e, "k_recon_inter4 (luma copy)" ) ) return st;
+    }
+    e = for_each_list( general_jobs, [&]( const aa_frame_list & l, int cnt ) {
+      LaunchTimer t( ctx, 0 ); ctx->stats.recon_inter_general_launches++; return aa::launch_recon_inter4( l, cnt, max_mbs, false, nullptr, ctx->compute ); } );
     if ( aa_status st = check( e, "k_recon_inter4" ) ) return st;
     if ( any_split ) {
       e = for_each_list( inter_jobs, [&]( const aa_frame_list & l, int cnt ) {
diff --git a/alfalfa_amd/csrc/runtime_submit.inc b/alfalfa_amd/csrc/runtime_submit.inc
--- a/alfalfa_amd/csrc/runtime_submit.inc
+++ b/alfalfa_amd/csrc/runtime_submit.inc
@@ -33,8 +33,10 @@
         intra_rows[r * words_per_row + ( col >> 6 )] |= 1ull << ( col & 63 );
       }
 
-  if ( !h.key_frame )
-    for ( size_t i = 0; i < nmb; i++ ) if ( mbs[i].y_mode == 9  ) { rec.has_split = true; break; }
+  if ( !h.key_frame ) {
+    const unsigned marks = aa_frame_marks_of_records( mbs, nmb );
+    rec.has_split = ( marks & AA_FRAME_HAS_SPLIT ) != 0; rec.frac_luma = ( marks & AA_FRAME_FRACTIONAL_LUMA ) != 0;
+  }
 
   fill_job( rec, job );
   job->mbs = reinterpret_cast<const aa_mb_info *>( c->dev + off + job_bytes );
@@ -287,7 +289,7 @@
     for ( uint32_t r = 0; r < mbh; r++ ) for ( uint32_t c = 0; c < mbw; c++ ) {
       const aa_mb_info & mb = mbs[r * mbw + c];
       if ( !( mb.flags & AA_MB_INTER ) ) rows[r * words_per_row + ( c >> 6 )] |= 1ull << ( c & 63 );
-      else if ( mb.y_mode == aa::SPLITMV ) split = 1;
+      else split |= aa::summary_marks_of( mb );
     }
     uint8_t * dense = nullptr;
     const size_t dense_bytes = align_up( std::max<size_t>( size_t( blocks ) * 32, 32 ) );
diff --git a/alfalfa_amd/csrc/runtime_types.inc b/alfalfa_amd/csrc/runtime_types.inc
--- a/alfalfa_amd/csrc/runtime_types.inc
+++ b/alfalfa_amd/csrc/runtime_types.inc
@@ -94,6 +94,7 @@
   int ref_after[3] = { -1, -1, -1 };
   std::vector<uint8_t> intra_diagonals;
   bool has_split = false;
+  bool frac_luma = false;
   bool handle_held = true;
   int chunk = -1;
   Batch * batch = nullptr;
diff --git a/alfalfa_amd/csrc/tok_fsm.hh b/alfalfa_amd/csrc/tok_fsm.hh
--- a/alfalfa_amd/csrc/tok_fsm.hh
+++ b/alfalfa_amd/csrc/tok_fsm.hh
@@ -24,6 +24,13 @@
   uint32_t done;
   uint32_t packed_words;
 };
+enum : uint32_t { SUM_HAS_SPLIT = 1, SUM_FRAC_LUMA = 2 };
+AA_HD inline uint32_t summary_marks_of( const aa_mb_info & mb )
+{
+  if ( !( mb.flags & AA_MB_INTER ) ) return 0;
+  if ( mb.y_mode == SPLITMV ) return SUM_HAS_SPLIT;
+  return ( ( mb.u.mv[0][0] | mb.u.mv[0][1] ) & 7 ) ? SUM_FRAC_LUMA : 0u;
+}
 enum : uint32_t { TOK_OK = 0, TOK_STEP_BOUND = 1, TOK_NO_MEMORY = 2,
                   TOK_HOST_FAILED = 3 };
 
diff --git a/alfalfa_amd/decoder.py b/alfalfa_amd/decoder.py
--- a/alfalfa_amd/decoder.py
+++ b/alfalfa_amd/decoder.py
@@ -375,6 +375,11 @@
         capi.check(self.L.aa_stream_frame_header(self.h, frame_index, C.byref(hdr)))
         return hdr.as_dict()
 
+    def frame_marks(self, frame_index):
+        bits = C.c_uint(0)
+        capi.check(self.L.aa_stream_frame_marks(self.h, frame_index, C.byref(bits)))
+        return bool(bits.value & 1), bool(bits.value & 2)
+
     def read_records(self, frame_index):
         h = self.frame_header(frame_index)
         mbw, mbh = h["mb_width"], h["mb_height"]
@@ -491,6 +496,12 @@
     def import_reference_host(self, y, u, v):
         y, u, v = (np.ascontiguousarray(p, dtype=np.uint8) for p in (y, u, v))
         capi.check(self.L.aa_stream_import_reference_host(self.h, y.ctypes.data_as(C.c_void_p), u.ctypes.data_as(C.c_void_p), v.ctypes.data_as(C.c_void_p)))
+
+
+def frame_marks_of_records(mb):
+    mb = np.ascontiguousarray(mb, dtype=MB_INFO_DTYPE).reshape(-1)
+    bits = capi.lib().aa_frame_marks_of_records(mb.ctypes.data_as(C.c_void_p), mb.size)
+    return bool(bits & 1), bool(bits & 2)
 
 
 def psnr(sse, width, height, planes):
diff --git a/include/alfalfa_amd.h b/include/alfalfa_amd.h
--- a/include/alfalfa_amd.h
+++ b/include/alfalfa_amd.h
@@ -160,6 +160,10 @@
 aa_status aa_submit_frames_ex( aa_ctx * ctx, const aa_frame_in * frames, int n, int * frame_index_out, int threads, unsigned flags );
 aa_status aa_launch_tokens( aa_ctx * ctx, int max_batches, int * launched_out );
 aa_status aa_stream_frame_header( aa_stream * s, int frame_index, aa_frame_header * out );
+#define AA_FRAME_HAS_SPLIT 1u
+#define AA_FRAME_FRACTIONAL_LUMA 2u
+aa_status aa_stream_frame_marks( aa_stream * s, int frame_index, unsigned * out );
+unsigned aa_frame_marks_of_records( const aa_mb_info * mbs, size_t n );
 aa_status aa_stream_read_records( aa_stream * s, int frame_index, aa_mb_info * mb_out, int16_t * coeff_out, size_t coeff_capacity_blocks );
 
 aa_status aa_stream_set_error_concealment( aa_stream * s, int on );
@@ -246,6 +250,7 @@
   uint64_t packed_frames, packed_words, packed_blocks;
   double host_batch_ms, host_batch_parse_wall_ms, host_batch_parse_cpu_ms, host_batch_arena_ms;
   uint64_t pinned_allocs;
+  uint64_t recon_inter_copy_launches, recon_inter_general_launches;
 } aa_kernel_stats;
 aa_status aa_ctx_profile( aa_ctx * ctx, int enable );
 aa_status aa_ctx_kernel_stats( aa_ctx * ctx, aa_kernel_stats * out, int reset );
```

After: 124.3 million. 1.9% lower.
